# PASSIONLab/ELBA

Hardware: AMD Instinct MI355X
Metric: overlap nnz/sec (A·Aᵀ SpGEMM, SharedSeeds semiring, after Prune(numshared<=1)) (higher is better)
Workload: dtype u32

## Files before the change

elba_amd/csrc/capi.hip:

```cpp
#include "common.hpp"
#include "ov_plan.hpp"
#include <new>

using namespace elba;

struct elba_ctx {
    Ctx c;
};

namespace {

template <class F>
int guarded(elba_ctx *ctx, F &&f)
{
    if (!ctx) return ELBA_ERR_INVALID_ARG;
    try {
        ELBA_HIP(hipSetDevice(ctx->c.device));
        f(ctx->c);
        return ELBA_OK;
    } catch (const Error &e) {
        ctx->c.last_error = e.msg;
        return e.code;
    } catch (const std::bad_alloc &) {
        ctx->c.last_error = "host allocation failed";
// ... 685 lines not shown

int elba_export_kmer_matrix(elba_ctx *ctx, elba_kmer_matrix_t *out)
{
    return guarded(ctx, [&](Ctx &c) {
        ELBA_REQUIRE(out, ELBA_ERR_INVALID_ARG, "export_kmer_matrix: null output");
        memset(out, 0, sizeof(*out));
        ELBA_REQUIRE(has(c.v, P_A), ELBA_ERR_STATE, "export_kmer_matrix: no k-mer matrix");
        const size_t M = (size_t)c.M, N = (size_t)c.N, Z = (size_t)c.Z;
        auto rp = download<uint32_t>(c, c.a_rowptr.p, M + 1);
        auto cp = download<uint32_t>(c, c.a_colptr.p, N + 1);
        auto csr = download<uint64_t>(c, c.a_csr.p, Z);
        auto csc = download<uint64_t>(c, c.a_csc.p, Z);
        out->nrows = c.M; out->ncols = c.N; out->nnz = c.Z;
        out->colptr = host_alloc<int64_t>(N + 1); out->rowptr = host_alloc<int64_t>(M + 1);
        out->csc_row = host_alloc<int64_t>(Z); out->csc_val = host_alloc<uint32_t>(Z);
        out->csr_col = host_alloc<int64_t>(Z); out->csr_val = host_alloc<uint32_t>(Z);
        for (size_t i = 0; i <= N; ++i) out->colptr[i] = cp[i];
        for (size_t i = 0; i <= M; ++i) out->rowptr[i] = rp[i];
        for (size_t z = 0; z < Z; ++z) {
            out->csc_row[z] = (int64_t)(csc[z] >> 32) + c.first_global_id_rows(); out->csc_val[z] = (uint32_t)csc[z];
            out->csr_col[z] = (int64_t)(csr[z] >> 32); out->csr_val[z] = (uint32_t)csr[z] & (c.csr_suffix ? 0xFFFFu : (c.csr_hints ? 0x3FFFFFFFu : 0xFFFFFFFFu));
        }
        if (c.csr_inline) {
            std::vector<size_t> fill(rp.begin(), rp.end() - 1);
            for (size_t k = 0; k < N; ++k)
                for (size_t z = cp[k]; z < cp[k + 1]; ++z) { const size_t at = fill[(size_t)(csc[z] >> 32)]++; out->csr_col[at] = (int64_t)k; out->csr_val[at] = (uint32_t)csc[z]; }
        }
        if (c.A_has_kmers) {
            out->kmers = host_alloc<uint64_t>(N);
            if (N) ELBA_HIP(hipMemcpyAsync(out->kmers, c.rel_kmers.p, N * 8, hipMemcpyDeviceToHost, c.stream));
            if (c.cfg.k > 32) {
                out->kmers_lo = host_alloc<uint64_t>(N);
                if (N) ELBA_HIP(hipMemcpyAsync(out->kmers_lo, c.rel_kmers_lo.p, N * 8, hipMemcpyDeviceToHost, c.stream));
            }
            if (c.cfg.k > 64) {
                out->kmers_lo2 = host_alloc<uint64_t>(N);
                if (N) ELBA_HIP(hipMemcpyAsync(out->kmers_lo2, c.rel_kmers_lo2.p, N * 8, hipMemcpyDeviceToHost, c.stream));
            }
            ELBA_HIP(hipStreamSynchronize(c.stream));
        }
    });
}

void elba_free_kmer_matrix(elba_kmer_matrix_t *m)
{
    if (!m) return;
    free(m->kmers); free(m->kmers_lo); free(m->kmers_lo2); free(m->colptr); free(m->csc_row); free(m->csc_val); free(m->rowptr); free(m->csr_col); free(m->csr_val);
    memset(m, 0, sizeof(*m));
}

int elba_kmer_histogram(elba_ctx *ctx, int64_t *hist, int64_t len)
{
    return guarded(ctx, [&](Ctx &c) {
        ELBA_REQUIRE(hist && len > 0, ELBA_ERR_INVALID_ARG, "kmer_histogram: null output");
        ELBA_REQUIRE(has(c.v, P_A), ELBA_ERR_STATE, "kmer_histogram: no k-mer matrix");
        auto cp = download<uint32_t>(c, c.a_colptr.p, (size_t)c.N + 1);
        for (int64_t i = 0; i < len; ++i) hist[i] = 0;
        for (int64_t k = 0; k < c.N; ++k) { int64_t n = (int64_t)cp[(size_t)k + 1] - cp[(size_t)k]; if (n < len) hist[n]++; }
    });
}

int elba_get_device_view(elba_ctx *ctx, elba_device_view *v)
{
    return guarded(ctx, [&](Ctx &c) {
        ELBA_REQUIRE(v, ELBA_ERR_INVALID_ARG, "get_device_view: null output");
        memset(v, 0, sizeof(*v));
        v->stream = (void *)c.stream;
        if (has(c.v, P_A)) { v->M = c.M; v->N = c.N; v->Z = c.Z; v->a_rowptr = c.a_rowptr.p; v->a_csr = c.a_csr.p; v->a_colptr = c.a_colptr.p; v->a_csc = c.a_csc.p;
                        v->a_csr_format = c.csr_inline ? ELBA_CSR_INLINE : (c.csr_suffix ? ELBA_CSR_DENSE : (c.csr_hints ? ELBA_CSR_HINTS : ELBA_CSR_PLAIN));
                        v->a_csr_pos_mask = c.csr_suffix ? 0xFFFFu : (c.csr_hints ? 0x3FFFFFFFu : 0xFFFFFFFFu);
                        v->a_kmers = c.A_has_kmers ? c.rel_kmers.p : nullptr;
                        v->a_gather_slots = c.use_ell && c.ell_compact ? c.ell_nslots : 0;
                        v->a_slot_kid = c.use_ell && c.ell_compact ? c.ell_slot_kid.p : nullptr; }
        if (has(c.v, P_B)) { v->Y = c.Y; v->b_rowptr = c.b_rowptr.p; v->b_col = c.b_col.p; v->b_val = c.b_val.p; }
    });
}

int elba_set_option(elba_ctx *ctx, const char *name, int64_t value)
{
    return guarded(ctx, [&](Ctx &c) {
        ELBA_REQUIRE(name, ELBA_ERR_INVALID_ARG, "set_option: null name");
        struct { const char *n; bool *b; } flags[] = {
            {"overlap_cold_calls", &c.cold_calls}, {"no_symmetry", &c.opt.no_symmetry}, {"no_ell", &c.opt.no_ell}, {"no_pay", &c.opt.no_pay}, {"mir32", &c.opt.mir32},
            {"no_hints", &c.opt.no_hints}, {"no_sample", &c.opt.no_sample}, {"no_slab", &c.opt.no_slab}, {"no_ell_compact", &c.opt.no_ell_compact}, {"msd_no_rank", &c.opt.msd_no_rank}, {"msd_rank", &c.opt.msd_rank}, {"csr_pairs_late", &c.opt.csr_pairs_late}, {"no_suffix", &c.opt.no_suffix}, {"ov_generic", &c.opt.ov_generic}, {"no_row_order", &c.opt.no_row_order}, {"no_inline", &c.opt.no_inline}, {"panel_inline", &c.opt.panel_inline}, {"kmer_pairs", &c.opt.kmer_pairs},
            {"kmer_unfused", &c.opt.kmer_unfused}, {"kmer_no_msd", &c.opt.kmer_no_msd}, {"kmer_msd", &c.opt.kmer_msd}, {"csr_pairs", &c.opt.csr_pairs}, {"emit_plain", &c.opt.emit_plain}, {"trace", &c.opt.trace}, {"measure_prep", &c.opt.measure_prep}};
        for (auto &f : flags) if (!strcmp(name, f.n)) { *f.b = value != 0; return; }
        if (!strcmp(name, "kmer_drop")) { ELBA_REQUIRE(value >= 0 && value <= 3, ELBA_ERR_INVALID_ARG, "set_option: kmer_drop is 0..3"); c.opt.kmer_drop = (int)value; }
        else if (!strcmp(name, "dense_up")) { ELBA_REQUIRE(value >= 0 && value <= 3, ELBA_ERR_INVALID_ARG, "set_option: dense_up is 0..3"); c.opt.dense_up = (int)value; }
        else if (!strcmp(name, "dense_wgs")) { ELBA_REQUIRE(value >= 1 && value <= 16, ELBA_ERR_INVALID_ARG, "set_option: dense_wgs is 1..16"); c.opt.dense_wgs = (int)value; }
        else if (!strncmp(name, "tune", 4) && name[4] >= '1' && name[4] <= '7' && name[4] != '6' && name[5] == 0) c.opt.tune[name[4] - '0'] = value;
        else if (!strcmp(name, "msd_small_cap")) c.opt.msd_small_cap = (int)value;
        else if (!strcmp(name, "kmer_batch_instances")) { ELBA_REQUIRE(value >= 0, ELBA_ERR_INVALID_ARG, "set_option: kmer_batch_instances is >= 0"); c.opt.kmer_batch_instances = value; }
        else if (!strcmp(name, "msd_wide_bits")) c.opt.msd_wide_bits = (int)value;
        else if (!strcmp(name, "ell_slot_cap")) c.opt.ell_slot_cap = (int)value;
        else if (!strcmp(name, "slab_pct")) { ELBA_REQUIRE(value >= 1 && value <= 1000, ELBA_ERR_INVALID_ARG, "set_option: slab_pct is 1..1000"); c.opt.slab_pct = (int)value; }
        else if (!strcmp(name, "slab_q16")) { ELBA_REQUIRE(value >= 0 && value < (1ll << 31), ELBA_ERR_INVALID_ARG, "set_option: slab_q16 is 0..2^31"); c.opt.slab_q16 = (int)value; }
        else if (!strcmp(name, "dk")) { ELBA_REQUIRE(value == -1 || value == 0 || value == 1 || value == 2 || value == 4, ELBA_ERR_INVALID_ARG, "set_option: dk is -1 (chosen per matrix), 0, 1, 2 or 4"); c.opt.dk = (int)value; }
        else if (!strcmp(name, "aln_tiers")) { ELBA_REQUIRE(value >= 0, ELBA_ERR_INVALID_ARG, "set_option: aln_tiers is a string of the digits 1, 2, 4, 8"); c.opt.aln_tiers = value; }
        else if (!strcmp(name, "aln_wide_hint")) c.opt.aln_wide_hint = (int)value;
        else if (!strcmp(name, "aln_long_hint")) c.opt.aln_long_hint = (int)value;
        else if (!strcmp(name, "polish_trace_bytes")) { ELBA_REQUIRE(value >= 0, ELBA_ERR_INVALID_ARG, "set_option: polish_trace_bytes is >= 0"); c.opt.polish_trace_bytes = value; }
        else throw Error{ELBA_ERR_INVALID_ARG, std::string("set_option: unknown option ") + name};
    });
}

int elba_release_workspace(elba_ctx *ctx)
{
    return guarded(ctx, [&](Ctx &c) {
        ELBA_REQUIRE(!c.dist_owner && c.ov_phase == 0, ELBA_ERR_STATE, "release_workspace: the context holds exchanged records or is inside a sharded multiplication");
        ELBA_HIP(hipStreamSynchronize(c.stream));
        c.ws_a.release(); c.ws_b.release(); c.ws_c.release(); c.ws_d.release(); c.ws_e.release(); c.ws_f.release(); c.ws_g.release(); c.ws_h.release(); c.ws_sort.release();
        c.csr_words.release(); c.kid_of_entry.release();
        c.cg_ptr.release(); c.cg_slot.release(); c.cg_kdeg.release(); c.cg_term.release(); c.cg_vinfo.release(); c.cg_ctr.release();
        c.cg_flag.release(); c.cg_cidx.release(); c.cg_nel.release(); c.cg_eoff.release();
        c.gl_ptr.release(); c.gl_bits.release(); c.gl_cnt.release(); c.gl_off.release(); c.gl_ctr.release(); c.gl_part.release(); c.gl_out.release();
        c.pl_cstart.release(); c.pl_cstrand.release(); c.pl_best.release(); c.pl_rec.release(); c.pl_clen.release(); c.pl_cred.release(); c.pl_ctr.release();
        c.pl_k0.release(); c.pl_k1.release(); c.pl_eptr.release(); c.pl_head.release(); c.pl_hidx.release(); c.pl_delta.release(); c.pl_dsum.release(); c.pl_gstart.release();
        c.pl_tok.release(); c.pl_tpos.release(); c.pl_seg_off.release(); c.pl_seg_start.release(); c.pl_seg_depth.release();
        c.po_plan.release(); c.po_rec.release(); c.po_toff.release(); c.po_trace.release(); c.po_col.release(); c.po_gap.release(); c.po_cnt.release();
        c.po_emit.release(); c.po_off.release(); c.po_cstat.release(); c.po_seq.release(); c.po_seqoff.release(); c.po_ctr.release();
        for (int b = 0; b < 2; ++b) { c.cg_far[b].release(); c.cg_rank[b].release(); c.cg_mn[b].release(); c.cg_cfar[b].release(); c.cg_crank[b].release(); }
        c.pu_k0.release(); c.pu_k1.release(); c.pu_eptr.release(); c.pu_head.release(); c.pu_hidx.release(); c.pu_delta.release();
        c.pu_dsum.release(); c.pu_gstart.release(); c.pu_tok.release(); c.pu_tpos.release(); c.pu_sel.release(); c.pu_rows.release(); c.pu_cols.release(); c.pu_vals.release();
        c.tm_cnt.release(); c.tm_bytes.release(); c.tm_first.release(); c.tm_boff.release(); c.tm_srcb.release();
        c.sg.release();
        c.tp_ntips.release(); c.tp_anchor.release();
        c.bb_end.release(); c.bb_len.release();
        c.wk_best.release(); c.wk_cnt.release(); c.wk_nweak.release(); c.wk_after.release();
        c.br_flank.release();
        c.sr_word.release();
        if (has(c.v, P_COUNTS)) { c.pre_ready = false; c.pre_consumed = true; }
    });
}

int elba_get_stat(elba_ctx *ctx, const char *name, int64_t *value)
{
    return guarded(ctx, [&](Ctx &c) {
        ELBA_REQUIRE(name && value, ELBA_ERR_INVALID_ARG, "get_stat: null name or value");
        if (!strcmp(name, "overlap_mirror_placed")) *value = c.ov_mir_placed;
        else if (!strcmp(name, "overlap_slab_q16")) *value = (int64_t)c.ov_slab_q16_used;
        else if (!strcmp(name, "kmer_path")) *value = c.kmer_path;
        else if (!strcmp(name, "kmer_passes")) *value = c.kmer_passes;
        else if (!strcmp(name, "kmer_crowded_buckets")) *value = c.kmer_crowded;
        else if (!strcmp(name, "kmer_crowded_small")) *value = c.kmer_crowded_small;
        else if (!strcmp(name, "kmer_largest_pass")) *value = c.kmer_largest_pass;
        else if (!strcmp(name, "kmer_peak_bytes")) *value = c.kmer_peak_bytes;
        else if (!strcmp(name, "kmer_buckets")) *value = c.kmer_buckets;
        else if (!strcmp(name, "overlap_passes")) *value = c.ov_passes;
        else if (!strcmp(name, "overlap_spec")) *value = c.ov_spec;
        else if (!strcmp(name, "overlap_forwarded")) *value = c.ov_forwarded;
        else if (!strncmp(name, "overlap_tier_limit_", 19) && name[19] >= '0' && name[19] < '0' + NUM_LDS_TIERS && !name[20]) *value = c.ov_tier_limit[name[19] - '0'];
        else if (!strncmp(name, "overlap_tier_queued_", 20) && name[20] >= '0' && name[20] < '0' + NUM_TIERS && !name[21]) *value = c.ov_tier_queued[name[20] - '0'];
        else if (!strncmp(name, "overlap_tier_done_", 18) && name[18] >= '0' && name[18] < '0' + NUM_TIERS && !name[19]) *value = c.ov_tier_done[name[18] - '0'];
        else if (!strcmp(name, "overlap_sort_rows_bucket")) *value = c.ov_sort_rows[0];
        else if (!strcmp(name, "overlap_sort_rows_huge")) *value = c.ov_sort_rows[1];
        else if (!strcmp(name, "overlap_family")) *value = c.ov_family;
        else if (!strcmp(name, "overlap_pay16")) *value = c.ov_pay16;
        else if (!strcmp(name, "overlap_rec16")) *value = c.ov_rec16_used;
        else if (!strcmp(name, "matrix_col_stride")) *value = has(c.v, P_A) && c.use_ell ? (int64_t)c.s_stride : 0;
        else if (!strcmp(name, "matrix_fbits")) *value = has(c.v, P_A) ? (int64_t)c.fbits : 0;
        else if (!strcmp(name, "matrix_pos16")) *value = has(c.v, P_A) && c.pos16 ? 1 : 0;
        else if (!strcmp(name, "matrix_hints")) *value = has(c.v, P_A) && c.csr_hints ? 1 : 0;
        else if (!strcmp(name, "matrix_inline")) *value = has(c.v, P_A) && c.csr_inline ? 1 : 0;
        else if (!strcmp(name, "matrix_suffix")) *value = has(c.v, P_A) && c.csr_suffix ? 1 : 0;
        else if (!strcmp(name, "matrix_csr_words")) *value = has(c.v, P_A) && c.csr_one_word ? 1 : 0;
        else if (!strcmp(name, "spgemm_prep_us")) *value = c.prep_us;
        else if (!strcmp(name, "emit_us")) *value = c.emit_us;
        else if (!strcmp(name, "triples_path")) *value = c.triples_path;
        else if (!strcmp(name, "text_tile_bytes")) *value = TEXT_TILE_BYTES;
        else if (!strcmp(name, "text_scan_span")) *value = scan_block_span();
        else if (!strcmp(name, "padded_columns")) *value = has(c.v, P_A) && c.use_ell ? 1 : 0;
        else if (!strcmp(name, "gather_slots")) *value = has(c.v, P_A) && c.use_ell ? c.ell_nslots : 0;
        else if (!strcmp(name, "contig_count")) *value = has(c.v, P_S, P_CONTIGS) ? c.cstats.contigs : 0;
        else if (!strcmp(name, "contig_cycles")) *value = has(c.v, P_S, P_CONTIGS) ? c.cstats.cycles : 0;
        else if (!strcmp(name, "contig_circular")) *value = has(c.v, P_S, P_CONTIGS) ? c.cg_circular : 0;
        else if (!strcmp(name, "contig_singletons")) *value = has(c.v, P_S, P_CONTIGS) ? c.cg_singletons : 0;
        else if (!strcmp(name, "contig_reads")) *value = has(c.v, P_S, P_CONTIGS) ? c.cstats.contig_reads : 0;
        else if (!strcmp(name, "contig_bases")) *value = has(c.v, P_S, P_CONTIGS) ? c.cstats.bases : 0;
        else if (!strcmp(name, "contig_branches")) *value = has(c.v, P_S, P_CONTIGS) ? c.cstats.branches : 0;
        else if (!strncmp(name, "graph_", 6)) {
            const bool ok = has(c.v, P_S, P_CONTIGS) && c.gl_for == c.cg_serial;
            const elba_graph_stats &g = c.gstats;
            const char *f = name + 6;
            int64_t x;
            if (!strcmp(f, "segments")) x = g.segments; else if (!strcmp(f, "candidates")) x = g.candidates; else if (!strcmp(f, "links")) x = g.links;
            else if (!strcmp(f, "closures")) x = g.closures; else if (!strcmp(f, "twisted")) x = g.twisted; else if (!strcmp(f, "unplaced")) x = g.unplaced;
            else if (!strcmp(f, "clamped")) x = g.clamped; else if (!strcmp(f, "asymmetric")) x = g.asymmetric;
            else throw Error{ELBA_ERR_INVALID_ARG, std::string("get_stat: unknown counter ") + name};
            *value = ok ? x : 0;
        }
        else if (!strncmp(name, "place_", 6)) {
            const bool ok = has(c.v, P_S, P_CONTIGS) && c.pl_for == c.cg_serial && c.pl_for != 0;
            const elba_place_stats &g = c.plstats;
            const char *f = name + 6;
            int64_t x;
            if (!strcmp(f, "chain")) x = g.chain; else if (!strcmp(f, "anchored")) x = g.anchored; else if (!strcmp(f, "unanchored")) x = g.unanchored;
            else if (!strcmp(f, "skipped")) x = g.skipped; else if (!strcmp(f, "candidates")) x = g.candidates; else if (!strcmp(f, "clipped")) x = g.clipped;
            else if (!strcmp(f, "outside")) x = g.outside; else if (!strcmp(f, "wrapped")) x = g.wrapped; else if (!strcmp(f, "segments")) x = g.segments;
            else if (!strcmp(f, "max_depth")) x = g.max_depth;
            else throw Error{ELBA_ERR_INVALID_ARG, std::string("get_stat: unknown counter ") + name};
            *value = ok ? x : 0;
        }
        else if (!strncmp(name, "polish_", 7)) {
            const bool ok = has(c.v, P_S, P_CONTIGS) && c.po_for == c.cg_serial && c.po_for != 0;
            const elba_polish_stats &g = c.postats;
            const char *f = name + 7;
            int64_t x;
            if (!strcmp(f, "voted")) x = g.voted; else if (!strcmp(f, "rejected")) x = g.rejected; else if (!strcmp(f, "outside")) x = g.outside;
            else if (!strcmp(f, "low_depth_columns")) x = g.low_depth_columns; else if (!strcmp(f, "bases_before")) x = g.bases_before;
            else if (!strcmp(f, "bases_after")) x = g.bases_after; else if (!strcmp(f, "sum_dist")) x = g.sum_dist; else if (!strcmp(f, "cells")) x = g.cells;
            else if (!strcmp(f, "batches")) x = g.batches;
            else throw Error{ELBA_ERR_INVALID_ARG, std::string("get_stat: unknown counter ") + name};
            *value = ok ? x : 0;
        }
        else if (!strcmp(name, "contig_rank_us")) *value = has(c.v, P_S, P_CONTIGS) ? (int64_t)(c.cstats.ms_rank * 1000.0f) : -1;
        else if (!strcmp(name, "resident_bytes_A")) {
            int64_t b = 0;
            if (has(c.v, P_A)) {
                b = (int64_t)(c.M + 1) * 4 + (int64_t)(c.N + 1) * 4 + 16 * c.Z;
                if (c.use_ell) b += 8 * c.ell_nslots * (int64_t)c.s_stride + (c.ell_compact ? 4 * c.ell_nslots : 0);
                if (c.csr_suffix) b += (4ll * c.N) << c.j_shift;
            }
            *value = b;
        }
        else throw Error{ELBA_ERR_INVALID_ARG, std::string("get_stat: unknown counter ") + name};
    });
}

int elba_kmer_hash_owner(elba_ctx *ctx, const uint64_t *kmers, int64_t n, int nprocs, uint64_t *hash, int32_t *owner)
{
    return guarded(ctx, [&](Ctx &c) { stage_ref_hash_owner(c, kmers, n, nprocs, hash, owner); });
}
// ... 133 lines not shown
```

elba_amd/csrc/common.hpp:

```cpp
#pragma once
#include <hip/hip_runtime.h>
#include <cstdint>
#include <cstdio>
#include <cstdlib>
#include <cstring>
#include <mutex>
#include <string>
#include <vector>
#include "../../include/elba_amd.h"
#include "state.hpp"
#include "msd_plan.hpp"

namespace elba {

struct Error {
    int code;
    std::string msg;
};

#define ELBA_HIP(expr)                                                                                   \
    do {                                                                                                 \
        hipError_t e__ = (expr);                                                                         \
        if (e__ != hipSuccess) {                                                                         \
            throw ::elba::Error{e__ == hipErrorOutOfMemory ? ELBA_ERR_OUT_OF_MEMORY : ELBA_ERR_HIP,      \
// ... 41 lines not shown
        if (e != hipSuccess) { want = bytes; e = hipMalloc(&p, want); }
        if (e != hipSuccess) { p = nullptr; throw Error{ELBA_ERR_OUT_OF_MEMORY, "hipMalloc of " + std::to_string(bytes) + " bytes failed"}; }
        cap = want;
    }
    void reserve_exact(size_t bytes)
    {
        if (bytes <= cap) return;
        release();
        const hipError_t e = hipMalloc(&p, bytes);
        if (e != hipSuccess) { p = nullptr; throw Error{ELBA_ERR_OUT_OF_MEMORY, "hipMalloc of " + std::to_string(bytes) + " bytes failed"}; }
        cap = bytes;
    }
    template <class T> T *as() const { return reinterpret_cast<T *>(p); }
    void swap(DevBuf &o) { void *tp = p; p = o.p; o.p = tp; size_t tc = cap; cap = o.cap; o.cap = tc; }
};

struct EventTimer {
    hipEvent_t a = nullptr, b = nullptr;
    void init() { if (!a) { ELBA_HIP(hipEventCreate(&a)); ELBA_HIP(hipEventCreate(&b)); } }
    void start(hipStream_t s) { init(); ELBA_HIP(hipEventRecord(a, s)); }
    void stop(hipStream_t s) { ELBA_HIP(hipEventRecord(b, s)); }
    float ms() { float t = 0; ELBA_HIP(hipEventSynchronize(b)); ELBA_HIP(hipEventElapsedTime(&t, a, b)); return t; }
    ~EventTimer() { if (a) (void)hipEventDestroy(a); if (b) (void)hipEventDestroy(b); }
};

template <int N>
struct PhaseMarks {
    hipEvent_t e[N] = {};
    void mark(int k, hipStream_t s) { if (!e[k]) ELBA_HIP(hipEventCreate(&e[k])); ELBA_HIP(hipEventRecord(e[k], s)); }
    float ms(int from, int to) { float t = 0; ELBA_HIP(hipEventSynchronize(e[to])); ELBA_HIP(hipEventElapsedTime(&t, e[from], e[to])); return t; }
    ~PhaseMarks() { for (int k = 0; k < N; ++k) if (e[k]) (void)hipEventDestroy(e[k]); }
};

void exclusive_scan_u32(hipStream_t s, const uint32_t *in, uint32_t *out, int64_t n, DevBuf &tmp);
void exclusive_scan_u32_to_i64(hipStream_t s, const uint32_t *in, int64_t *out, int64_t n, DevBuf &tmp);
__device__ __forceinline__ uint32_t column_hint(const uint64_t *col, uint32_t L, uint32_t i, uint32_t win_lo, uint32_t win_hi)
{
    bool own_g = false, own_w = false;
    uint32_t mult = 0;
    for (uint32_t t = 0; t < L; ++t) {
        const uint32_t j = (uint32_t)(col[t] >> 32);
        if (j == i) { ++mult; continue; }
        const bool par = ((i ^ j) & 1u) ? j < i : j > i;
        own_g |= par; own_w |= par || j < win_lo || j >= win_hi;
    }
    if (mult >= 2) return 0u;
    return (own_g ? 0u : 1u) | (own_w ? 0u : 2u);
}

int radix_sort_pairs(hipStream_t s, uint64_t *k0, uint64_t *v0, uint64_t *k1, uint64_t *v1, int64_t n, int bit_lo, int bit_hi, DevBuf &tmp);
int radix_sort_keys(hipStream_t s, uint64_t *k0, uint64_t *k1, int64_t n, int bit_lo, int bit_hi, DevBuf &tmp, bool first_hist_done = false);
int radix_sort_where(int64_t n, int bit_lo, int bit_hi);
struct CsrFin { int idbits, pb, rs, mb, pbi; uint64_t *csr; uint32_t *rowptr; int64_t M; };
void radix_sort_keys_to_csr(hipStream_t s, uint64_t *k0, uint64_t *k1, int64_t n, const CsrFin &f, DevBuf &tmp);
int radix_sort_pairs_k32(hipStream_t s, uint32_t *k0, uint64_t *v0, uint32_t *k1, uint64_t *v1, int64_t n, int bit_lo, int bit_hi, DevBuf &tmp);
void group_offsets_k32(hipStream_t s, const uint32_t *sorted_keys, int64_t n, uint32_t *ptr, int64_t nkeys);
void radix_column_scan(hipStream_t s, uint32_t *rows, int64_t nrows, uint32_t nbins, DevBuf &tmp);
uint32_t *radix_first_histogram(int64_t n, int bit_lo, int bit_hi, DevBuf &tmp, int *shift, int *bits, int *tile);
void fill_u32(hipStream_t s, uint32_t *p, uint32_t v, int64_t n);
void fill_u64(hipStream_t s, uint64_t *p, uint64_t v, int64_t n);
void group_offsets_u32(hipStream_t s, const uint64_t *sorted_keys, int key_shift, int64_t n, uint32_t *ptr, int64_t nkeys);
uint64_t reduce_max_u64(hipStream_t s, const uint64_t *p, int64_t n, DevBuf &tmp);
int64_t scan_block_span();

struct Options {
    bool no_symmetry = false;
    bool no_ell = false;
    bool no_pay = false;
    bool mir32 = false;
    bool no_hints = false;
    bool no_sample = false;
    bool no_ell_compact = false;
    bool no_slab = false;
    bool csr_pairs_late = false;
    bool msd_rank = false;
    bool msd_no_rank = false;
    int ell_slot_cap = 0;
    int slab_pct = 175;
    int slab_q16 = 0;
    bool panel_inline = false;
    bool no_inline = false;
    bool no_suffix = false;
    bool ov_generic = false;
    bool no_row_order = false;
    bool kmer_pairs = false;
    bool kmer_unfused = false;
    bool kmer_msd = false;
    bool kmer_no_msd = false;
    bool csr_pairs = false;
    bool emit_plain = false;
    bool trace = false;
    bool measure_prep = false;
    int64_t tune[8] = {0, 0, 0, 0, 0, 0, 0, 0};
    int msd_wide_bits = 0;
    int64_t kmer_batch_instances = 0;
    int msd_small_cap = 0;
    int kmer_drop = 0;
    int dense_up = 1;
    int dense_wgs = 8;
    int dk = -1;
    int64_t aln_tiers = 0;
    int aln_wide_hint = 6, aln_long_hint = 6000;
    int64_t polish_trace_bytes = 0;
};

struct RowWindow { int64_t lo, hi; int64_t rows() const { return hi - lo; } };

struct alignas(16) SymEntry { uint32_t col; int32_t suffix, suffixT; uint32_t meta; };
static_assert(sizeof(SymEntry) == 16, "tr.hip and stars.hip read 16-byte entries");

struct Ctx {
    elba_cfg cfg{};
    Options opt;
    int device = 0;
    hipStream_t stream = nullptr;
    std::string last_error;
    int num_cus = 256;
    Validity v;

    int64_t nreads = 0, first_global_id = 0, packed_bytes = 0;
    const uint8_t *d_packed = nullptr;
    const uint64_t *d_byte_off = nullptr;
    const uint32_t *d_len = nullptr;
    DevBuf own_packed, own_byte_off, own_len;
    uint32_t max_read_len = 0;
    std::vector<uint32_t> h_len;
    std::vector<uint64_t> h_byte_off;
    bool tx_index = false;
    DevBuf tx_recs, tx_name_pos, tx_name_len;
    std::vector<elba_fasta_record_t> tx_h_recs; std::vector<uint64_t> tx_h_name_pos; std::vector<uint32_t> tx_h_name_len;

    int triples_path = 0;
    int kmer_passes = 1;
    int64_t kmer_crowded = 0, kmer_crowded_small = 0, kmer_largest_pass = 0;
    int64_t kmer_peak_bytes = 0;
    int64_t kmer_buckets = 0;
    int kmer_path = 0;
    int64_t I = 0, ndistinct = 0;
    DevBuf inst_off;
    DevBuf rel_kmers;
    DevBuf rel_kmers_lo;
    DevBuf rel_kmers_lo2;
    DevBuf rel_counts;
    DevBuf csr_words;
    bool pre_pairs = false;
    bool pre_ready = false, pre_consumed = false, pre_words = false, pre_hints = false, pre_hints_done = false, pre_ell_done = false, pre_inline = false, pre_inline_pending = false ; int pre_rs = 0, pre_pbi = 0; int pre_nb = 0, pre_pb = 0; uint64_t pre_maxpos = 0;
    bool csr_hints = false, ov_hints_used = false, ov_rec16 = false;
    bool csr_inline = false;
    bool csr_inline_window = false;
    bool csr_one_word = false;
    bool csr_suffix = false;
    DevBuf ov_sample;
    int64_t A_products = 0;
    DevBuf prod_ctr;
    DevBuf kid_of_entry;
    elba_kmer_stats kstats{};

    bool A_has_kmers = false;
    int64_t M = 0, N = 0, Z = 0, max_row_nnz = 0, max_col_nnz = 0;
    DevBuf a_rowptr, a_csr, a_colptr, a_csc;
    DevBuf a_ell;
    bool use_ell = false;
    bool ell_compact = false;
    int64_t ell_nslots = 0, ell_cap_cols = 0;
    DevBuf ell_slot_kid;
    DevBuf a_ellj;
// ... 32 lines not shown
    DevBuf tr_in_rows, tr_in_cols, tr_in_vals;
    int64_t tr_M = 0, tr_nnz = 0, tr_id_base = 0;
    DevBuf tr_deg, tr_pas, tr_flags, tr_k0, tr_v0, tr_k1, tr_v1, tr_ptr, tr_sym, tr_src, tr_mark, tr_ctr, tr_sel, tr_out_rows, tr_out_cols, tr_out_vals;
    int64_t tr_sym_M = 0, tr_sym_n = 0;
    elba_string_stats sstats{};

    int64_t cg_n = 0, cg_E = 0, cg_bases = 0, cg_circular = 0, cg_singletons = 0;
    DevBuf cg_ptr, cg_slot, cg_kdeg, cg_far[2], cg_rank[2], cg_mn[2], cg_term, cg_vinfo, cg_flag, cg_cidx, cg_nel, cg_eoff, cg_ctr;
    DevBuf cg_cid, cg_eread, cg_epre, cg_estr, cg_eboff, cg_soff, cg_coff, cg_seq, cg_kind;
    DevBuf cg_cfar[2], cg_crank[2];
    EventTimer cg_t_total, cg_t_rank;
    elba_contig_stats cstats{};

    DevBuf gl_ptr, gl_bits, gl_cnt, gl_off, gl_ctr, gl_part, gl_out;
    EventTimer gl_t_total;
    elba_graph_stats gstats{};
    uint64_t cg_serial = 0, gl_for = 0;

    int64_t pu_M = 0, pu_n = 0, pu_nseg = 0;
    DevBuf pu_k0, pu_k1, pu_eptr, pu_head, pu_hidx, pu_delta, pu_dsum, pu_gstart, pu_tok, pu_tpos, pu_ctr, pu_sel, pu_rows, pu_cols, pu_vals;
    DevBuf pu_seg_off, pu_seg_start, pu_seg_depth, pu_trim, pu_flags;
    EventTimer pu_t_total;
    elba_pileup_stats pustats{};
    elba_pileup_cfg pu_cfg{};

    DevBuf pl_cstart, pl_cstrand, pl_best, pl_rec, pl_clen, pl_cred, pl_ctr;
    DevBuf pl_k0, pl_k1, pl_eptr, pl_head, pl_hidx, pl_delta, pl_dsum, pl_gstart, pl_tok, pl_tpos, pl_seg_off, pl_seg_start, pl_seg_depth;
    EventTimer pl_t_total;
    elba_place_stats plstats{};
    uint64_t pl_for = 0;

    DevBuf po_plan, po_rec, po_toff, po_trace, po_col, po_gap, po_cnt, po_emit, po_off, po_cstat, po_seq, po_seqoff, po_ctr;
    EventTimer po_t_total, po_t_align;
    elba_polish_stats postats{};
    uint64_t po_for = 0;

    int64_t tm_n = 0, tm_packed_bytes = 0;
    DevBuf tm_packed, tm_off, tm_len, tm_src, tm_beg, tm_end;
    DevBuf tm_cnt, tm_bytes, tm_first, tm_boff, tm_srcb, tm_ctr;
    EventTimer tm_t_total, tm_t_repack;
    elba_trim_stats tmstats{};

    struct SgWork {
        DevBuf ptr, removed, keep, pos, st, rows, cols, vals;
        EventTimer t_total, t_compact;
        void release() { ptr.release(); removed.release(); keep.release(); pos.release(); st.release(); rows.release(); cols.release(); vals.release(); }
    } sg;

    DevBuf tp_ntips, tp_anchor;
    elba_tip_stats tpstats{};

    DevBuf bb_end, bb_len;
    elba_bubble_stats bbstats{};

    DevBuf wk_best, wk_cnt, wk_nweak, wk_after;
    elba_weak_stats wkstats{};

    DevBuf br_flank;
    elba_bridge_stats brstats{};

    DevBuf sr_word;
    elba_star_stats srstats{};

    DevBuf ws_scan, ws_sort, ws_a, ws_b, ws_c, ws_d, ws_e, ws_f;
    DevBuf ws_cursor;
    DevBuf ws_g, ws_h;
    DevBuf ov_totcnt, ov_mir, ov_tmp, ov_sum_tmp;
    bool ov_low_clean = false;
    DevBuf ov_rowcnt, ov_rowoff, ov_lists, ov_counters, ov_gtable, ov_sortkeys;
    int64_t ov_tmp_cap = 0;
    bool ov_sort_used[2] = {false, false};
    bool ov_tiers_known = false, ov_tier_used[8] = {false, false, false, false, false, false, false, false};
    int64_t b_cap_entries = 0;
    uint64_t ov_calls = 0;
    uint32_t ov_prior_q16 = 0;
    uint32_t ov_slab_q16 = 0;
    DevBuf ov_slab;
    int64_t ov_slab_cap = 0;
    DevBuf ov_tickrows;
    DevBuf ov_slabpos, ov_slabn;
    bool ov_slab_on = false;
    uint32_t ov_slab_q16_used = 0;
    int64_t ov_mir_placed = 0;
    int64_t ov_spec = 0;
    int64_t ov_tier_limit[5] = {0, 0, 0, 0, 0}, ov_tier_queued[6] = {0, 0, 0, 0, 0, 0}, ov_tier_done[6] = {0, 0, 0, 0, 0, 0}, ov_sort_rows[2] = {0, 0};
    int64_t ov_family = 0, ov_pay16 = 0, ov_rec16_used = 0;
    int64_t ov_passes = 0, ov_forwarded = 0;
    int ov_phase = 0;
    int ov_pend_passes = 1; bool ov_pend_timed = false; float ov_pend_ms[3] = {0, 0, 0};
    std::vector<uint64_t> ov_remote_bounds;
    DevBuf ov_remote;
    int64_t ov_send_slot = 0;
    DevBuf ov_cursors;
    bool own_stream = true;

    EventTimer t_total, t_a, t_b, t_c;
    EventTimer t_emit, t_emit_plain; int64_t prep_us = -1, emit_us = -1;
    struct PinnedHost { void *p = nullptr; size_t cap = 0; void reserve(size_t n) { if (n <= cap) return; if (p) (void)hipHostFree(p); p = nullptr; cap = 0; ELBA_HIP(hipHostMalloc(&p, n, hipHostMallocDefault)); cap = n; } ~PinnedHost() { if (p) (void)hipHostFree(p); } };
    PinnedHost ov_host;
    PhaseMarks<5> ov_marks;
};

inline void reads_replaced(Ctx &c, Event ev)
{
    done(c.v, ev);
    if (c.A_has_kmers) done(c.v, EV_MATRIX_OF_OLD_READS);
    c.tx_index = false;
}

struct GraphInput { int64_t M, n, id_base; const int64_t *rows, *cols; const elba_overlap_t *vals; };
inline GraphInput graph_input(Ctx &c, const char *who)
{
    if (has(c.v, P_EDGES)) return {c.tr_in_M, c.tr_in_n, 0, c.tr_in_rows.as<int64_t>(), c.tr_in_cols.as<int64_t>(), c.tr_in_vals.as<elba_overlap_t>()};
    ELBA_REQUIRE(has(c.v, P_ALN), ELBA_ERR_STATE, std::string(who) + ": no overlaps (call elba_align_seeds or elba_set_overlaps)");
    ELBA_REQUIRE(c.row_hi < 0 || (c.row_lo == 0 && c.row_hi == c.M), ELBA_ERR_STATE,
                 std::string(who) + ": this context aligned a row shard; gather the ranks' overlaps and load them with elba_set_overlaps");
    return {c.M, c.naln, c.first_global_id_rows(), c.aln_rows.as<int64_t>(), c.aln_cols.as<int64_t>(), c.aln_out.as<elba_overlap_t>()};
}

struct ReadSource { const uint8_t *packed; const uint64_t *byte_off; const uint32_t *len; bool replicated; };
inline ReadSource read_source(Ctx &c, int64_t M, const char *who, const char *what, bool take_replicated = true)
{
    if (take_replicated && c.aln_all_n == M && c.aln_all_n >= 0) return {c.aln_all_packed.as<uint8_t>(), c.aln_all_off.as<uint64_t>(), c.aln_all_len.as<uint32_t>(), true};
    if (has(c.v, P_READS) && c.nreads == M) return {c.d_packed, c.d_byte_off, c.d_len, false};
    std::string w(what);
    w.replace(w.find('#'), 1, std::to_string(M));
    throw Error{ELBA_ERR_STATE, std::string(who) + ": the " + w + " are not on this context (elba_set_reads or elba_dist_set_all_reads)"};
}

struct DepthBufs { DevBuf &k0, &k1, &eptr, &head, &hidx, &delta, &dsum, &gstart, &tok, &tpos, &seg_off, &seg_start, &seg_depth; };
void depth_reserve(const DepthBufs &b, int64_t max_keys, int64_t G);
const uint64_t *depth_segments(Ctx &c, const DepthBufs &b, int64_t E, int64_t M, int mb, int pb, const uint32_t *len, unsigned long long *ctr);

constexpr int PLACE_CTR_BAD = 2, PLACE_CTR_WORDS = 16;
struct PlaceWork { GraphInput in; ReadSource src; int64_t M, base, E, nc; elba_placement_t *rec; unsigned long long *ctr; const uint32_t *clen; };
PlaceWork place_records(Ctx &c, int skip_flags, const char *who, bool depth_bufs, EventTimer *t);
[[noreturn]] void place_throw_bad_pair(Ctx &c, const PlaceWork &w, int64_t a, const char *who);

void stage_set_reads_fasta(Ctx &c, const char *chunk, int64_t chunk_bytes, uint64_t chunk_file_offset, const elba_fasta_record_t *recs, int64_t nreads,
                           int64_t first_global_id, elba_ingest_stats *stats);
void launch_fasta_encode(Ctx &c, const uint8_t *d_chunk, uint64_t chunk_file_offset, uint64_t chunk_bytes, const elba_fasta_record_t *d_recs, const uint64_t *d_byte_off,
                         int64_t nreads, uint8_t *d_packed);
constexpr uint32_t TEXT_TILE_BYTES = 4096;
void stage_set_reads_text(Ctx &c, const char *chunk, int64_t chunk_bytes, uint64_t chunk_file_offset, const elba_text_cfg *cfg, elba_text_stats *stats);
void stage_export_read_index(Ctx &c, elba_fasta_record_t *recs, uint64_t *name_pos, uint32_t *name_len, int64_t nreads_capacity);
void stage_count_kmers(Ctx &c);
void stage_create_kmer_matrix(Ctx &c);
bool msd_matrix_from_triples(Ctx &c, int64_t M, int64_t N, int64_t Z, const int64_t *d_rows, const int64_t *d_cols, const uint32_t *d_vals);
bool msd_count_kmers(Ctx &c, uint64_t I, elba_kmer_stats &st);
void choose_column_store(Ctx &c, int64_t N, int64_t max_col);
void stage_set_kmer_matrix(Ctx &c, int64_t M, int64_t N, int64_t Z, const int64_t *rows, const int64_t *cols, const uint32_t *vals);
void stage_set_kmer_matrix_device(Ctx &c, int64_t M, int64_t N, int64_t Z, const int64_t *d_rows, const int64_t *d_cols, const uint32_t *d_vals);
void stage_export_triples_device(Ctx &c, int64_t *d_rows, int64_t *d_cols, uint32_t *d_vals);
void stage_create_seed_matrix(Ctx &c);
void stage_seed_matrix_begin(Ctx &c, int nranks, const uint64_t *bounds_host, uint64_t *send_counts_host);
void stage_seed_matrix_fill(Ctx &c, void *d_send, const uint64_t *offsets_host);
void stage_seed_matrix_end(Ctx &c, const void *d_recv, int64_t nrecv);
void stage_seed_matrix_send(Ctx &c, int nranks, const uint64_t *bounds_host, void *d_send, int64_t slot);
bool stage_seed_matrix_recv(Ctx &c, void *d_recv, int64_t slot, int64_t *slot_needed);
void stage_align_seeds(Ctx &c, int mat, int mis, int gap, int dropoff);
void stage_dist_set_all_reads(Ctx &c, const void *d_packed, int64_t packed_bytes, const void *d_byte_off, const void *d_len, int64_t nreads_total);
void stage_set_overlaps(Ctx &c, int64_t nreads, const int64_t *rows, const int64_t *cols, const elba_overlap_t *vals, int64_t n);
void stage_transitive_reduction(Ctx &c, double bad_read_cutoff, int fuzz);
void stage_generate_contigs(Ctx &c, int flags);
void stage_generate_contigs_ex(Ctx &c, const elba_contig_cfg *cfg);
void stage_export_assembly_links(Ctx &c, elba_links_t *out);
// ... 28 lines not shown
```

elba_amd/csrc/ov_plan.hpp:

```cpp
#pragma once
#include <algorithm>
#include <cstddef>
#include <cstdint>

namespace elba {

constexpr int NUM_LDS_TIERS = 5;
constexpr int NUM_TIERS = NUM_LDS_TIERS + 1;
constexpr int LDS_TBITS0 = 9;
constexpr uint32_t STAGE_CHUNK = 1024;
constexpr uint32_t STAGE_REC_BYTES = 32;
constexpr uint32_t FIN_WAVE2_MAX = 1024;
constexpr uint32_t SLAB_PAD = 16;
constexpr int RP_TILE = 1024;
constexpr int FIN_HUGE_BLOCKS = 32;
constexpr int OV_SAMPLE_ROWS = 256, OV_SAMPLE_TIER = 3;
constexpr size_t OV_LDS_MAX = 160 * 1024;

namespace ov_spec {
constexpr uint32_t half = 1, inl = 1, pay16 = 1, rec16 = 1, suffix = 0, qblk_log2 = 0, j_shift = 0;
constexpr uint32_t hint_mask = 1u << 31, pos_mask = 0x3FFFFFFFu;
}

enum OvFamily { OV_DENSE, OV_PAY, OV_S32, OV_SHARED };
constexpr int OV_GRID_DENSE_WGS = 0, OV_GRID_SPILL = -1;
struct OvTierRow { OvFamily family; int tier, block, tbits, tbc, cu_factor, slot_bytes; bool global, payload, dense; int dense_up_min; };
constexpr OvTierRow OV_ROWS[] = {
    {OV_DENSE, 0, 256, 9, 9, OV_GRID_DENSE_WGS, 18, false, false, true, 0},
    {OV_DENSE, 1, 256, 10, 0, 4, 18, false, false, true, 0},
    {OV_DENSE, 1, 512, 10, 10, 4, 18, false, false, true, 1},
    {OV_DENSE, 2, 512, 11, 0, 2, 18, false, false, true, 0},
    {OV_DENSE, 2, 1024, 11, 11, 2, 18, false, false, true, 2},
    {OV_DENSE, 3, 1024, 12, 0, 1, 18, false, false, true, 0},
    {OV_PAY, 0, 128, 9, 0, 9, 26, false, true, false, 0},
    {OV_PAY, 1, 256, 10, 0, 4, 26, false, true, false, 0},
    {OV_PAY, 2, 512, 11, 0, 2, 26, false, true, false, 0},
    {OV_PAY, 3, 1024, 12, 0, 1, 26, false, true, false, 0},
    {OV_S32, 0, 128, 9, 0, 12, 18, false, false, false, 0},
    {OV_S32, 1, 256, 10, 0, 7, 18, false, false, false, 0},
    {OV_S32, 2, 512, 11, 0, 3, 18, false, false, false, 0},
    {OV_S32, 3, 1024, 12, 0, 1, 18, false, false, false, 0},
    {OV_SHARED, 4, 256, 13, 0, 1, 18, false, false, false, 0},
    {OV_SHARED, NUM_LDS_TIERS, 256, 0, 0, OV_GRID_SPILL, 0, true, false, false, 0},
};
constexpr int OV_NROWS = (int)(sizeof(OV_ROWS) / sizeof(OV_ROWS[0]));

constexpr int64_t ov_stage_slack(int num_cus) { return (int64_t)num_cus * 32 * STAGE_CHUNK + 64; }

constexpr size_t ov_row_lds(const OvTierRow &r, bool pay16)
{
    const size_t waves = (size_t)(r.block / 64), table = r.global ? 0 : (size_t)r.slot_bytes << r.tbits;
    return table + 256 + waves * (r.dense ? 2368 : r.global ? 2560 : r.payload ? 3072 : pay16 ? 2048 : 2560);
}

inline int ov_row_of(OvFamily family, int tier, int dense_up)
{
    int found = -1;
    for (int r = 0; r < OV_NROWS; ++r) {
        const OvTierRow &x = OV_ROWS[r];
        if (x.tier == tier && (x.family == family || x.family == OV_SHARED) && dense_up >= x.dense_up_min) found = r;
    }
    return found;
}

struct OvOptions {
    bool no_symmetry = false, no_pay = false, mir32 = false, no_slab = false, no_sample = false, ov_generic = false;
    int dk = -1, dense_up = 1, dense_wgs = 8, slab_q16 = 0, slab_pct = 175;
    int64_t tune3 = 0, tune4 = 0, tune5 = 0, tune7 = 0;
};
struct OvHints { uint32_t prior_q16 = 0, slab_q16 = 0; bool tiers_known = false, tier_used[NUM_TIERS] = {false, false, false, false, false, false}, sort_used[2] = {false, false}; };
struct OvInput {
    int64_t M = 0, N = 0, Z = 0, row_lo = 0, row_hi = 0, max_row_nnz = 0, max_col_nnz = 0;
    uint32_t fbits = 1;
    bool pos16 = false, use_ell = false, csr_hints = false, csr_inline = false, csr_suffix = false, have_row_order = false;
    int num_cus = 256;
    OvOptions opt;
    OvHints hints;
    int phase = 0, pass = 1;
    int64_t tmp_cap = 0, free_bytes = 0, workspace_hint_bytes = 0;
};

struct OvLaunch { int row = -1, grid = 0, block = 0; size_t lds = 0; };
struct OvFinPlan {
    int64_t nrows = 0;
    bool slabs = false, scan_rowptr = false, narrow = false;
    int slab_fold_blocks = 0, rowptr_blocks = 0, row_blocks = 0, bucket_blocks = 0, huge_blocks = FIN_HUGE_BLOCKS;
    uint64_t sort_stride = 2;
    uint32_t sorts = 0;
};
struct OvPlan {
    int64_t nrows = 0;
    bool whole = false, ell = false, forced = false;
    uint32_t half = 0, pos_mask = 0, hint_mask = 0, suffix = 0, inl = 0;
    bool row_order = false, hints_used = false;
    bool pay = false, pay16 = false;
    OvFamily family = OV_S32;
    int dk = 1;
    bool spec = false;
    uint32_t min_tier = 0, qblk_log2 = 0, prior_q16 = 16384, use_feedback = 1, max_col = 1;
    unsigned long long fb_enough = 0;
    uint32_t nsample = 0, sstep = 1;
    bool slab_on = false; int64_t slab_cap = 0; uint32_t slab_prior_q16 = 0;
    uint64_t gstride = 2; int spill_blocks = 64;
    int64_t slack = 0, tmp_cap = 0, b_cap = 0;
    bool mir16 = false;
    uint32_t tier_limit[NUM_LDS_TIERS] = {0, 0, 0, 0, 0};
    OvLaunch tier[NUM_TIERS], sample;
    int tmax = NUM_TIERS;
    uint32_t launched = 0;
    int zero_blocks_max = 0, classify_blocks = 0;
    OvFinPlan fin;
};

inline bool ov_spec_ok(const OvPlan &p)
{
    return !p.forced && p.dk == 0 && !p.pay && (p.pay16 ? 1u : 0u) == ov_spec::pay16 && p.ell && p.half == ov_spec::half && p.hint_mask == ov_spec::hint_mask &&
           p.pos_mask == ov_spec::pos_mask && p.inl == ov_spec::inl && (p.mir16 ? 1u : 0u) == ov_spec::rec16 && p.suffix == ov_spec::suffix && !p.row_order &&
           p.qblk_log2 == ov_spec::qblk_log2 && p.whole;
}

inline OvLaunch ov_launch_of(int row, bool pay16, int num_cus, int dense_wgs, int spill_blocks)
{
    const OvTierRow &r = OV_ROWS[row];
    OvLaunch l;
    l.row = row; l.block = r.block; l.lds = ov_row_lds(r, pay16);
    l.grid = r.cu_factor == OV_GRID_SPILL ? spill_blocks : num_cus * (r.cu_factor == OV_GRID_DENSE_WGS ? dense_wgs : r.cu_factor);
    return l;
}

inline OvFinPlan plan_ov_finalize(const OvInput &in, bool slabs, bool all_sorts, bool remote)
{
    OvFinPlan f;
    const int64_t M = in.M, cus = in.num_cus;
    f.nrows = in.row_hi - in.row_lo;
    f.slabs = slabs;
    f.slab_fold_blocks = slabs && f.nrows > 0 ? (int)((f.nrows + 255) / 256) : 0;
    while (f.sort_stride < (uint64_t)M) f.sort_stride <<= 1;
    f.scan_rowptr = M + 1 > (1 << 17);
    f.rowptr_blocks = (int)(f.scan_rowptr ? (M + 1 + 255) / 256 : (M + 1 + RP_TILE - 1) / RP_TILE);
    if (f.nrows <= 0) return f;
    f.row_blocks = (int)std::min<int64_t>((f.nrows + 3) / 4, cus * 32);
    f.narrow = in.opt.tune4 != 2 && !remote &&
               std::min<uint64_t>((uint64_t)std::max<int64_t>(in.max_row_nnz, 1) * (uint64_t)std::max<int64_t>(in.max_col_nnz, 1), (uint64_t)M) <= (uint64_t)FIN_WAVE2_MAX;
    f.bucket_blocks = (int)std::min<int64_t>(f.nrows, cus * 4);
    if (!f.narrow && (all_sorts || in.hints.sort_used[0])) f.sorts |= 1u;
    if (!f.narrow && (all_sorts || in.hints.sort_used[1])) f.sorts |= 2u;
    return f;
}

inline bool ov_one_triangle(const OvInput &in) { return in.phase >= 1 || !in.opt.no_symmetry || in.csr_inline; }

struct OvSpill { uint64_t gstride; int blocks; };
inline OvSpill ov_spill_tables(int64_t M, int num_cus)
{
    OvSpill s{2, 0};
    while (s.gstride < 2ull * (uint64_t)(M > 1 ? M : 1)) s.gstride <<= 1;
    s.blocks = (int)((4ull << 30) / (20ull * s.gstride));
    s.blocks = s.blocks < 64 ? 64 : (s.blocks > num_cus * 2 ? num_cus * 2 : s.blocks);
    return s;
}

inline void ov_plan_capacities(const OvInput &in, OvPlan &p)
{
    const int64_t M = in.M, Z = in.Z;
    const bool half = ov_one_triangle(in);
    const OvSpill sp = ov_spill_tables(M, in.num_cus);
    p.gstride = sp.gstride; p.spill_blocks = sp.blocks;
    p.slack = ov_stage_slack(in.num_cus);
    p.tmp_cap = in.tmp_cap;
    if (p.tmp_cap == 0) {
        if (in.workspace_hint_bytes > 0) p.tmp_cap = in.workspace_hint_bytes / (int64_t)STAGE_REC_BYTES;
        else {
            const int64_t budget = (int64_t)((size_t)in.free_bytes / 2 / (STAGE_REC_BYTES + (half ? 2 * (24 + 32) : 24)));
            p.tmp_cap = std::min<int64_t>(std::max<int64_t>(half ? Z / 2 : Z, 1 << 16) + p.slack, std::max<int64_t>(budget, 1024));
        }
        if (p.tmp_cap < 1024) p.tmp_cap = 1024;
    }
    p.b_cap = half ? 2 * p.tmp_cap : p.tmp_cap;
}

inline void ov_plan_switches(const OvInput &in, OvPlan &p)
{
    const OvOptions &o = in.opt;
    const int64_t Z = in.Z, nrows = p.nrows;
    p.max_col = (uint32_t)(in.max_col_nnz > 0 ? in.max_col_nnz : 1);
    p.half = in.phase >= 1 ? 2u : (ov_one_triangle(in) ? 1u : 0u);
    p.pos_mask = in.csr_suffix ? 0xFFFFu : (in.csr_hints ? 0x3FFFFFFFu : 0xFFFFFFFFu);
    p.hint_mask = !in.csr_hints ? 0u : (p.half == 2u ? 1u << 30 : (p.half == 1u ? 1u << 31 : 0u));
    p.suffix = in.csr_suffix && p.half == 1u ? 1u : 0u;
    p.inl = in.csr_inline ? 1u : 0u;
    p.row_order = p.suffix && in.have_row_order;
    p.hints_used = p.hint_mask != 0u || p.suffix != 0u || in.csr_inline;
    p.prior_q16 = in.hints.prior_q16 ? in.hints.prior_q16 : 16384u;
    p.use_feedback = in.hints.prior_q16 ? 0u : 1u;
    p.fb_enough = (unsigned long long)std::min<int64_t>(std::max<int64_t>(Z / 32, 1 << 16), 1 << 23);
    p.pay = in.pos16 && !o.no_pay;
    p.pay16 = p.pay && in.use_ell && !in.csr_suffix && o.tune3 != 1 && ((uint64_t)in.max_row_nnz << in.fbits) <= 65536ull;
    if (p.pay16) p.pay = false;
    p.family = p.suffix ? OV_DENSE : p.pay ? OV_PAY : OV_S32;
    p.mir16 = in.pos16 && !o.mir32;
    p.qblk_log2 = o.tune5 > 0 ? (uint32_t)std::min<int64_t>(o.tune5 - 1, 12) : 0u;
    p.min_tier = (p.pay16 && nrows >= 65536 && Z / nrows >= 1024 && o.tune4 != 1) ? 2u : 0u;
    if (o.tune7 >= 1 && o.tune7 <= NUM_TIERS) p.min_tier = (uint32_t)(o.tune7 - 1);
    p.dk = o.dk >= 0 ? o.dk : ((in.csr_inline && in.N > 0 && Z < 3 * in.N) ? 0 : 1);
    p.spec = ov_spec_ok(p);
}

inline void ov_plan_sample_slabs(const OvInput &in, OvPlan &p)
{
    const OvOptions &o = in.opt;
    const int64_t M = in.M, nrows = p.nrows;
    const bool sampling = p.use_feedback && nrows >= 8192 && !o.no_sample;
    p.nsample = sampling ? (uint32_t)OV_SAMPLE_ROWS : 0u; p.sstep = sampling ? (uint32_t)(nrows / OV_SAMPLE_ROWS) : 1u;
    p.slab_prior_q16 = o.slab_q16 > 0 ? (uint32_t)o.slab_q16 : in.hints.slab_q16;
    p.slab_on = in.phase == 0 && p.half == 1u && p.mir16 && !o.no_slab && nrows > 0 && (sampling || p.slab_prior_q16 != 0u);
    if (p.slab_on) {
        p.slab_cap = std::min<int64_t>(p.tmp_cap + (int64_t)SLAB_PAD * nrows, 0xFFFF0000ll);
        if (p.slab_cap + M >= 0xFFFFFFFFll) p.slab_cap = std::max<int64_t>(0xFFFFFFFFll - M - 1, 0);
        if (p.slab_cap <= (int64_t)SLAB_PAD * nrows + 1) p.slab_on = false;
    }
}

inline void ov_plan_tiers(const OvInput &in, OvPlan &p)
{
    const OvOptions &o = in.opt;
    const int64_t M = in.M, nrows = p.nrows;
    for (int t = 0; t < NUM_TIERS; ++t) p.tier[t] = ov_launch_of(ov_row_of(p.family, t, (int)o.dense_up), p.pay16, in.num_cus, o.dense_wgs, p.spill_blocks);
    for (int t = 0; t < NUM_LDS_TIERS; ++t) {
        const uint32_t T = 1u << OV_ROWS[p.tier[t].row].tbits;
        p.tier_limit[t] = std::min((T >> 2) * 3, T - (uint32_t)p.tier[t].block) - 1;
    }
    if (p.nsample) p.sample = p.tier[OV_SAMPLE_TIER];
    if (o.tune4 != 2 && in.pass == 1) {
        const uint64_t ubm = std::min<uint64_t>((uint64_t)std::max<int64_t>(in.max_row_nnz, 1) * (uint64_t)p.max_col, (uint64_t)(uint32_t)M);
        const int gmax = ubm <= 1 ? 1 : 64 - __builtin_clzll(2 * ubm - 1);
        p.tmax = gmax <= LDS_TBITS0 ? 0 : gmax - LDS_TBITS0;
        p.tmax = std::max(p.tmax, (int)p.min_tier);
        if (p.suffix) p.tmax = std::max(p.tmax, (int)o.dense_up);
    }
    const bool all_tiers = !in.hints.tiers_known || in.phase == 2;
    for (int t = 0; t < NUM_TIERS; ++t)
        if (nrows > 0 && (all_tiers || in.hints.tier_used[t]) && t <= p.tmax) p.launched |= 1u << t;
}

inline OvPlan plan_ov(const OvInput &in)
{
    OvPlan p;
    const OvOptions &o = in.opt;
    const int64_t cus = in.num_cus, nrows = in.row_hi - in.row_lo;
    p.nrows = nrows;
    p.whole = in.row_lo == 0 && in.row_hi == in.M;
    p.ell = in.use_ell;
    p.forced = o.ov_generic || o.dk >= 0 || o.tune3 != 0 || o.tune4 != 0 || o.tune5 != 0 || o.tune7 != 0;
    ov_plan_capacities(in, p);
    ov_plan_switches(in, p);
    ov_plan_sample_slabs(in, p);
    ov_plan_tiers(in, p);
    p.zero_blocks_max = in.num_cus * 8;
    p.classify_blocks = nrows > 0 ? (int)std::min<int64_t>((nrows + 255) / 256, cus * 4) : 0;
    p.fin = plan_ov_finalize(in, p.half == 1u && p.mir16 && p.slab_on, !in.hints.tiers_known, false);
    return p;
}

inline OvInput ov_next_pass(const OvInput &in, const OvPlan &p, bool overflow, unsigned long long cursor)
{
    OvInput n = in;
    n.pass = in.pass + 1;
    n.tmp_cap = overflow ? (int64_t)cursor + p.slack : p.tmp_cap;
    n.hints.tiers_known = false;
    return n;
}

struct OvMeasured { int64_t Z = 0, nnz = 0, ndiag = 0, extra_nnz = 0; bool whole = false; unsigned long long fb_claims = 0, fb_ub = 0; unsigned int tier_count[NUM_TIERS] = {0, 0, 0, 0, 0, 0}, fin_count[2] = {0, 0}; };
inline OvHints ov_next_hints(const OvHints &old, const OvMeasured &m)
{
    OvHints h = old;
    for (int t = 0; t < NUM_TIERS; ++t) h.tier_used[t] = m.tier_count[t] > 0;
    h.tiers_known = true;
    h.sort_used[0] = m.fin_count[0] > 0; h.sort_used[1] = m.fin_count[1] > 0;
    if (m.whole && m.Z > 0 && m.extra_nnz == 0) {
        const double r = 0.5 * (double)(m.nnz - m.ndiag) / (double)m.Z * 65536.0;
        h.slab_q16 = r < 1.0 ? 1u : (r > 4.0e9 ? 4000000000u : (uint32_t)r);
    }
    if (m.fb_ub > 0) {
        const double r = 1.25 * (double)m.fb_claims / (double)m.fb_ub * 65536.0;
        const uint32_t q = r < 64.0 ? 64u : (r > 4.0e9 ? 4000000000u : (uint32_t)r);
        if (old.prior_q16 == 0 || q > old.prior_q16 + old.prior_q16 / 10 || q + old.prior_q16 / 10 < old.prior_q16) h.prior_q16 = q;
    }
    return h;
}

}
```

elba_amd/csrc/spgemm.hip:

```cpp
#include "common.hpp"
#include "ov_plan.hpp"
#include <algorithm>
#include <string>
#include <type_traits>
#include <utility>

namespace elba {

namespace {

constexpr uint32_t EMPTY = 0xFFFFFFFFu;
constexpr uint32_t FIN_WAVE_MAX = 256;
constexpr uint32_t FIN_LDS_MAX = 4096;

struct alignas(128) OvShard {
    unsigned long long yraw, nnz, ndiag, nupper, fb_claims, fb_ub, products;
    unsigned int maxshared;
    unsigned int tier_done[NUM_TIERS];
};
constexpr int NUM_SHARDS = 64;

struct OvCounters {
    unsigned long long cursor;
    unsigned long long products;
// ... 39 lines not shown
    uint32_t M;
    uint32_t Mcols;
    uint32_t row_lo, row_hi;
    uint32_t fbits;
    uint32_t half;
    uint32_t tier_limit[NUM_LDS_TIERS];
    uint32_t use_feedback;
    uint32_t prior_q16;
    uint32_t *row_cnt;
    uint32_t *low_cnt;
    unsigned long long *row_off;
    uint32_t *lists;
    const uint32_t *row_order, *row_label;
    uint32_t *sample_list; uint32_t nsample, sstep;
    uint32_t *fin_lists;
    OvCounters *ctr;
    StageRec *tmp; unsigned long long tmp_cap;
    uint32_t rec16; uint4 *rec; uint32_t *tick;
    uint32_t *gtable; unsigned long long gstride;
    uint4 *slab; unsigned long long slab_cap; uint32_t slab_prior_q16, slab_pct;
    unsigned long long *slab_pos;
};

struct OvSpecParams {
    static constexpr uint32_t half = ov_spec::half, inl = ov_spec::inl, pay16 = ov_spec::pay16, rec16 = ov_spec::rec16, suffix = ov_spec::suffix, qblk_log2 = ov_spec::qblk_log2, j_shift = ov_spec::j_shift;
    static constexpr uint32_t hint_mask = ov_spec::hint_mask, pos_mask = ov_spec::pos_mask;
    static constexpr uint32_t row_lo = 0, row_hi = 0xFFFFFFFFu;
    static constexpr const uint32_t *a_colptr = nullptr, *a_ellj = nullptr, *row_order = nullptr, *row_label = nullptr;
    static constexpr const uint64_t *a_csc = nullptr;
    static constexpr StageRec *tmp = nullptr;
    static constexpr uint32_t *gtable = nullptr;
    static constexpr unsigned long long gstride = 0;
    const uint32_t *a_rowptr; const uint64_t *a_csr; const uint64_t *a_ell;
    uint32_t *tick_rows;
    uint32_t s_stride, lpc_log2, max_col, fbits, M, Mcols, use_feedback;
    uint32_t tier_limit[NUM_LDS_TIERS];
    unsigned long long fb_enough, tmp_cap;
    uint32_t *row_cnt, *low_cnt; unsigned long long *row_off;
    uint32_t *lists, *sample_list;
    OvCounters *ctr;
    uint4 *rec; uint32_t *tick;
    uint4 *slab; unsigned long long *slab_pos;
};

struct ZeroList { uint32_t *p[6]; size_t words[6]; int n; };
__global__ __launch_bounds__(256) void k_zero_regions(ZeroList z)
{
    const size_t stride = (size_t)gridDim.x * 256u;
    for (int q = 0; q < z.n; ++q)
        for (size_t i = (size_t)blockIdx.x * 256u + threadIdx.x; i < z.words[q]; i += stride) z.p[q][i] = 0u;
}

struct __attribute__((packed, aligned(4))) RowPair { uint32_t a, b; };
__device__ __forceinline__ uint32_t slab_base(uint32_t rp, uint32_t rp0, uint32_t row_rel, uint32_t q16)
{
    return (uint32_t)(((unsigned long long)(rp - rp0) * q16) >> 16) + SLAB_PAD * row_rel;
}

__device__ __forceinline__ uint32_t wave_sum_u32(uint32_t v)
{
#pragma unroll
    for (int d = 32; d >= 1; d >>= 1) v += __shfl_xor(v, d, 64);
    return v;
}

__device__ __forceinline__ uint32_t guaranteed_tbits(uint32_t ub, uint32_t mcols)
{
    const uint32_t need = ub < mcols ? ub : mcols;
    return need <= 1 ? 1u : (uint32_t)(32 - __clz(2 * need - 1));
}

#include "spgemm_table.hpp"
#include "spgemm_direct.hpp"

struct FinParams {
    const uint32_t *row_cnt; uint32_t *low_cnt; const unsigned long long *row_off; int64_t *b_rowptr;
    const StageRec *tmp; StageRec *mir;
    uint32_t rec16; const uint4 *rec; const uint32_t *tick;
    uint32_t *b_col; elba_seed_t *b_val;
    uint32_t M, row_lo, row_hi, half;
    uint32_t *fin_lists; OvCounters *ctr;
    uint64_t *sortkeys; unsigned long long sort_stride;
    uint32_t *sum_tmp;
    long long b_cap;
    uint32_t mir16;
    const uint32_t *tick_rows;
    const uint32_t *a_rowptr; uint4 *slab;
    const unsigned long long *slab_pos; uint32_t *slab_n;
};

struct SlabCall { uint32_t q16, rp0; };
__device__ __forceinline__ SlabCall slab_call(const FinParams &p)
{
    SlabCall s{0u, 0u};
    if (p.slab) { s.q16 = p.ctr->slab_q16; if (s.q16) s.rp0 = p.a_rowptr[p.row_lo]; }
    return s;
}
__device__ __forceinline__ uint2 slab_row(const FinParams &p, const SlabCall &s, uint32_t i)
{
    if (!s.q16) return make_uint2(0u, 0u);
    return make_uint2(slab_base(p.a_rowptr[i], s.rp0, i - p.row_lo, s.q16), p.slab_n[i]);
}
__global__ void k_slab_fold(FinParams p)
{
    const uint32_t i = p.row_lo + blockIdx.x * blockDim.x + threadIdx.x;
    if (i >= p.row_hi) return;
    const SlabCall s = slab_call(p);
    uint32_t n = 0;
    if (s.q16) {
        const unsigned long long w = p.slab_pos[i];
        const uint32_t base = slab_base(p.a_rowptr[i], s.rp0, i - p.row_lo, s.q16), cur = (uint32_t)w, lim = (uint32_t)(w >> 32);
        n = (cur < lim ? cur : lim) - base;
    }
    p.slab_n[i] = n;
}

__device__ __forceinline__ void fin_load(const FinParams &p, uint32_t low, unsigned long long off, int64_t dst, uint32_t t, uint4 &a, uint4 &b, uint2 sl = make_uint2(0u, 0u))
{
    if (t >= low) {
        if (p.rec16) {
            const uint4 m = p.rec[off + (t - low)];
            a = make_uint4(m.x, 0xFFFFFFFFu, m.y & 0xFFFFu, m.y >> 16); b = make_uint4(m.z & 0xFFFFu, m.z >> 16, m.w, 0u);
        } else { const StageRec *r = &p.tmp[off + (t - low)]; a = r->a; b = r->b; }
    }
    else if (p.mir16) {
        const uint4 m = t < sl.y ? p.slab[sl.x + t] : reinterpret_cast<const uint4 *>(p.mir)[dst + t - sl.y];
        a = make_uint4(m.x, 0xFFFFFFFFu, m.y & 0xFFFFu, m.y >> 16); b = make_uint4(m.z & 0xFFFFu, m.z >> 16, m.w, 0u);
    } else { const StageRec *r = &p.mir[dst + t]; a = r->a; b = r->b; }
}
__device__ __forceinline__ uint32_t fin_col(const FinParams &p, uint32_t low, unsigned long long off, int64_t dst, uint32_t t, uint2 sl = make_uint2(0u, 0u))
{
    if (t >= low) return p.rec16 ? p.rec[off + (t - low)].x : p.tmp[off + (t - low)].a.x;
    return p.mir16 ? (t < sl.y ? p.slab[sl.x + t].x : reinterpret_cast<const uint4 *>(p.mir)[dst + t - sl.y].x) : p.mir[dst + t].a.x;
}
__device__ __forceinline__ elba_seed_t rec_seed(const uint4 a, const uint4 b)
{
    elba_seed_t v;
    v.q0 = a.z; v.t0 = a.w; v.q1 = b.x; v.t1 = b.y; v.numshared = (int32_t)b.z;
    return v;
}

__global__ __launch_bounds__(256) void k_row_pointers(FinParams p)
{
    __shared__ unsigned long long wsum[4], bsum;
    const uint32_t tid = threadIdx.x, lane = tid & 63, w = tid >> 6;
    const uint32_t n = p.M + 1, t0 = blockIdx.x * RP_TILE;
    unsigned long long pre = 0;
    {
        const uint4 *ca = reinterpret_cast<const uint4 *>(p.row_cnt), *cb = reinterpret_cast<const uint4 *>(p.low_cnt), *cc = reinterpret_cast<const uint4 *>(p.slab_n);
#pragma unroll 4
        for (uint32_t q = tid; q < t0 / 4; q += 256) {
            const uint4 x = ca[q], z = cb[q];
            pre += (unsigned long long)x.x + x.y + x.z + x.w + z.x + z.y + z.z + z.w;
            if (cc) { const uint4 y2 = cc[q]; pre += (unsigned long long)y2.x + y2.y + y2.z + y2.w; }
        }
    }
    uint32_t v[4];
    unsigned long long mine = 0;
#pragma unroll
    for (int u = 0; u < 4; ++u) {
        const uint32_t e = t0 + tid * 4 + u;
        v[u] = e < p.M ? p.row_cnt[e] + p.low_cnt[e] + (p.slab_n ? p.slab_n[e] : 0u) : 0u;
        mine += v[u];
    }
#pragma unroll
    for (int d = 32; d >= 1; d >>= 1) pre += __shfl_xor(pre, d, 64);
    unsigned long long inc = mine;
#pragma unroll
    for (int d = 1; d < 64; d <<= 1) { const unsigned long long o = __shfl_up(inc, d, 64); if ((int)lane >= d) inc += o; }
    if (lane == 63) wsum[w] = inc;
    if (tid == 0) bsum = 0;
    __syncthreads();
    if (lane == 0) atomicAdd(&bsum, pre);
    __syncthreads();
    unsigned long long run = bsum + inc - mine;
    for (uint32_t k = 0; k < w; ++k) run += wsum[k];
#pragma unroll
    for (int u = 0; u < 4; ++u) {
        const uint32_t e = t0 + tid * 4 + u;
        if (e < n) p.b_rowptr[e] = (int64_t)run;
        run += v[u];
    }
}

__global__ void k_sum_counts(FinParams p)
{
    const uint32_t e = blockIdx.x * blockDim.x + threadIdx.x;
    if (e <= p.M) p.sum_tmp[e] = e < p.M ? p.row_cnt[e] + p.low_cnt[e] + (p.slab_n ? p.slab_n[e] : 0u) : 0u;
}

__global__ __launch_bounds__(256) void k_mirror(FinParams p)
{
    const uint32_t lane = threadIdx.x & 63;
    const uint32_t wave = (blockIdx.x * blockDim.x + threadIdx.x) >> 6;
    const uint32_t nwaves = (gridDim.x * blockDim.x) >> 6;
    uint32_t placed = 0;
    for (uint32_t i = p.row_lo + wave; i < p.row_hi; i += nwaves) {
        const uint32_t own = p.row_cnt[i];
        const unsigned long long off = p.row_off[i];
        const uint32_t y = own + p.low_cnt[i] + (p.slab_n ? p.slab_n[i] : 0u);
        if (lane == 0 && y > FIN_WAVE2_MAX) {
            const int which = y > FIN_LDS_MAX ? 1 : 0;
            const uint32_t at = atomicAdd(&p.ctr->fin_count[which], 1u);
            p.fin_lists[(size_t)which * p.M + at] = i;
        }
        if (!p.half || p.rec16) continue;
        if (p.tick_rows && !((p.tick_rows[i >> 5] >> (i & 31u)) & 1u)) continue;
        for (uint32_t t = lane; t < own; t += 64) {
            const uint4 a = p.tmp[off + t].a;
            if (a.y == 0xFFFFFFFFu) continue;
            const uint4 b = p.tmp[off + t].b;
            const int64_t at = p.b_rowptr[a.x] + (int64_t)a.y;
            if (at >= p.b_cap) continue;
            if (p.mir16) reinterpret_cast<uint4 *>(p.mir)[at] = make_uint4(i, a.w | a.z << 16, b.y | b.x << 16, b.z);
            else {
                p.mir[at].a = make_uint4(i, 0xFFFFFFFFu, a.w, a.z);
                p.mir[at].b = make_uint4(b.y, b.x, b.z, 0u);
            }
        }
    }
    if (p.half && p.rec16) {
        const uint32_t n = p.ctr->ntick, stride = gridDim.x * blockDim.x;
        for (uint32_t e = blockIdx.x * blockDim.x + threadIdx.x; e < n; e += stride) {
            const uint32_t i = p.tick[3ull * e], t = p.tick[3ull * e + 1u], tk = p.tick[3ull * e + 2u];
            const uint4 r = p.rec[p.row_off[i] + t];
            const uint4 img = make_uint4(i, (r.y >> 16) | (r.y << 16), (r.z >> 16) | (r.z << 16), r.w);
            ++placed;
            const int64_t at = p.b_rowptr[r.x] + (int64_t)tk;
            if (at >= p.b_cap) continue;
            if (p.mir16) reinterpret_cast<uint4 *>(p.mir)[at] = img;
            else { p.mir[at].a = make_uint4(i, 0xFFFFFFFFu, img.y & 0xFFFFu, img.y >> 16); p.mir[at].b = make_uint4(img.z & 0xFFFFu, img.z >> 16, img.w, 0u); }
        }
    }
    placed = wave_sum_u32(placed);
    if (lane == 0 && placed) atomicAdd(&p.ctr->mir_placed, (unsigned long long)placed);
}

__global__ __launch_bounds__(256) void k_finalize_wave(FinParams p)
{
    __shared__ uint32_t colsm[4][FIN_WAVE_MAX];
    const int lane = threadIdx.x & 63, w = threadIdx.x >> 6;
    const uint32_t wave = (blockIdx.x * blockDim.x + threadIdx.x) >> 6;
    const uint32_t nwaves = (gridDim.x * blockDim.x) >> 6;
    uint32_t *cols = colsm[w];
    const SlabCall sc = slab_call(p);
    for (uint32_t i = p.row_lo + wave; i < p.row_hi; i += nwaves) {
        const int64_t dst = p.b_rowptr[i];
        const uint32_t y = (uint32_t)(p.b_rowptr[i + 1] - dst);
        const uint32_t lowt = p.low_cnt[i];
        if (lane == 0 && lowt) p.low_cnt[i] = 0;
        if (y == 0 || y > FIN_WAVE_MAX) continue;
        if (dst + (int64_t)y > p.b_cap) continue;
        const unsigned long long off = p.row_off[i];
        const uint2 sl = slab_row(p, sc, i);
        const uint32_t low = lowt + sl.y;
        uint32_t mine[4];
        uint4 ra[4], rb[4];
#pragma unroll
        for (int u = 0; u < 4; ++u) {
            const uint32_t t = (uint32_t)lane + 64u * u;
            mine[u] = 0xFFFFFFFFu;
            if (t < y) {
                fin_load(p, low, off, dst, t, ra[u], rb[u], sl);
                mine[u] = ra[u].x;
                cols[t] = mine[u];
            }
        }
        __builtin_amdgcn_fence(__ATOMIC_RELEASE, "wavefront");
        __builtin_amdgcn_wave_barrier();
        uint32_t rank[4] = {0, 0, 0, 0};
        for (uint32_t l = 0; l < y; ++l) {
            const uint32_t c = cols[l];
#pragma unroll
            for (int u = 0; u < 4; ++u) rank[u] += c < mine[u] ? 1u : 0u;
        }
#pragma unroll
        for (int u = 0; u < 4; ++u) {
            const uint32_t t = (uint32_t)lane + 64u * u;
            if (t < y) { p.b_col[dst + rank[u]] = mine[u]; p.b_val[dst + rank[u]] = rec_seed(ra[u], rb[u]); }
        }
        __builtin_amdgcn_wave_barrier();
    }
}

__global__ __launch_bounds__(256) void k_finalize_mid(FinParams p)
{
    __shared__ uint64_t lkeys[4][FIN_WAVE2_MAX];
    __shared__ uint32_t bst[4][128], bfl[4][128];
    const int lane = threadIdx.x & 63, w = threadIdx.x >> 6;
// ... 280 lines not shown
{
    uint32_t lo = 0, hi = p.nranks;
    while (hi - lo > 1) { const uint32_t mid = (lo + hi) >> 1; if (p.bounds[mid] <= read) lo = mid; else hi = mid; }
    return lo;
}
template <bool FILL>
__global__ __launch_bounds__(256) void k_remote_mirror(RemoteParams p, unsigned long long *cnt_or_cursor, StageRec *send)
{
    __shared__ uint32_t cnt[REMOTE_MAX_RANKS], fill[REMOTE_MAX_RANKS];
    __shared__ unsigned long long base[REMOTE_MAX_RANKS];
    const uint32_t tid = threadIdx.x, lane = tid & 63, w = tid >> 6;
    const uint32_t r0 = p.row_lo + blockIdx.x * REMOTE_ROWS_PER_BLOCK, r1 = min(r0 + (uint32_t)REMOTE_ROWS_PER_BLOCK, p.row_hi);
    if (tid < REMOTE_MAX_RANKS) { cnt[tid] = 0; fill[tid] = 0; }
    __syncthreads();
    for (uint32_t i = r0 + w; i < r1; i += 4) {
        const uint32_t n = p.row_cnt[i];
        const unsigned long long off = p.row_off[i];
        for (uint32_t t = lane; t < n; t += 64) {
            const uint32_t j = p.rec16 ? p.rec[off + t].x : p.tmp[off + t].a.x;
            if (j != i && (j < p.row_lo || j >= p.row_hi)) atomicAdd(&cnt[remote_rank_of(p, j)], 1u);
        }
    }
    __syncthreads();
    if (tid < p.nranks && cnt[tid]) {
        const unsigned long long b = atomicAdd(&cnt_or_cursor[tid], (unsigned long long)cnt[tid]);
        if (FILL) base[tid] = b;
    }
    if (!FILL) return;
    __syncthreads();
    for (uint32_t i = r0 + w; i < r1; i += 4) {
        const uint32_t n = p.row_cnt[i];
        const unsigned long long off = p.row_off[i];
        for (uint32_t t = lane; t < n; t += 64) {
            uint4 a, b = make_uint4(0u, 0u, 0u, 0u);
            if (p.rec16) { const uint4 m = p.rec[off + t]; a = make_uint4(m.x, 0u, m.y & 0xFFFFu, m.y >> 16); b = make_uint4(m.z & 0xFFFFu, m.z >> 16, m.w, 0u); }
            else a = p.tmp[off + t].a;
            const uint32_t j = a.x;
            if (j != i && (j < p.row_lo || j >= p.row_hi)) {
                if (!p.rec16) b = p.tmp[off + t].b;
                const uint32_t d = remote_rank_of(p, j);
                const unsigned long long at = base[d] + atomicAdd(&fill[d], 1u);
                send[at].a = make_uint4(j, i, a.w, a.z);
                send[at].b = make_uint4(b.y, b.x, b.z, 0u);
            }
        }
    }
}

__global__ void k_ingest_remote(StageRec *rem, unsigned long long n, uint32_t *low_cnt, uint32_t row_lo, uint32_t row_hi, unsigned long long *bad, unsigned long long *nupper)
{
    const unsigned long long r = (unsigned long long)blockIdx.x * blockDim.x + threadIdx.x;
    unsigned long long up = 0;
    if (r < n) {
        const uint32_t j = rem[r].a.x;
        if (j < row_lo || j >= row_hi) atomicAdd(bad, 1ull);
        else { rem[r].b.w = atomicAdd(&low_cnt[j], 1u); up = rem[r].a.y > j ? 1u : 0u; }
    }
#pragma unroll
    for (int d = 32; d >= 1; d >>= 1) up += __shfl_xor(up, d, 64);
    if ((threadIdx.x & 63) == 0 && up) atomicAdd(nupper, up);
}

__global__ void k_place_remote(FinParams p, const StageRec *rem, unsigned long long n, unsigned long long slot)
{
    if (slot) { rem += (unsigned long long)blockIdx.y * slot; n = (unsigned long long)rem->a.x + 1; if (n > slot) n = slot; }
    for (unsigned long long r = (unsigned long long)blockIdx.x * blockDim.x + threadIdx.x + (slot ? 1 : 0); r < n; r += (unsigned long long)gridDim.x * blockDim.x) {
        const uint4 a = rem[r].a, b = rem[r].b;
        if (a.x < p.row_lo || a.x >= p.row_hi) continue;
        const int64_t at = p.b_rowptr[a.x] + (int64_t)b.w;
        if (at >= p.b_cap) continue;
        if (p.mir16) reinterpret_cast<uint4 *>(p.mir)[at] = make_uint4(a.y, a.z | a.w << 16, b.x | b.y << 16, b.z);
        else { p.mir[at].a = make_uint4(a.y, 0xFFFFFFFFu, a.z, a.w); p.mir[at].b = make_uint4(b.x, b.y, b.z, 0u); }
    }
}


static bool ov_mir16(const Ctx &c) { return c.pos16 && !c.opt.mir32; }

static OvInput ov_input(Ctx &c, int phase, int pass)
{
    OvInput in;
    const RowWindow w = c.window();
    in.M = c.M; in.N = c.N; in.Z = c.Z; in.row_lo = w.lo; in.row_hi = w.hi; in.max_row_nnz = c.max_row_nnz; in.max_col_nnz = c.max_col_nnz;
    in.fbits = c.fbits; in.pos16 = c.pos16; in.use_ell = c.use_ell; in.csr_hints = c.csr_hints; in.csr_inline = c.csr_inline; in.csr_suffix = c.csr_suffix;
    in.have_row_order = c.have_row_order; in.num_cus = c.num_cus;
    const Options &o = c.opt;
    in.opt.no_symmetry = o.no_symmetry; in.opt.no_pay = o.no_pay; in.opt.mir32 = o.mir32; in.opt.no_slab = o.no_slab; in.opt.no_sample = o.no_sample; in.opt.ov_generic = o.ov_generic;
    in.opt.dk = o.dk; in.opt.dense_up = o.dense_up; in.opt.dense_wgs = o.dense_wgs; in.opt.slab_q16 = o.slab_q16; in.opt.slab_pct = o.slab_pct;
    in.opt.tune3 = o.tune[3]; in.opt.tune4 = o.tune[4]; in.opt.tune5 = o.tune[5]; in.opt.tune7 = o.tune[7];
    in.hints.prior_q16 = c.ov_prior_q16; in.hints.slab_q16 = c.ov_slab_q16; in.hints.tiers_known = c.ov_tiers_known;
    for (int t = 0; t < NUM_TIERS; ++t) in.hints.tier_used[t] = c.ov_tier_used[t];
    in.hints.sort_used[0] = c.ov_sort_used[0]; in.hints.sort_used[1] = c.ov_sort_used[1];
    in.phase = phase; in.pass = pass;
    in.tmp_cap = c.ov_tmp_cap; in.workspace_hint_bytes = c.cfg.workspace_hint_bytes;
    if (in.tmp_cap == 0 && in.workspace_hint_bytes <= 0) {
        size_t free_b = 0, total_b = 0;
        ELBA_HIP(hipMemGetInfo(&free_b, &total_b));
        in.free_bytes = (int64_t)free_b;
    }
    return in;
}

template <int R, int DK, bool SPEC> static constexpr auto ov_row_kernel()
{
    constexpr OvTierRow r = OV_ROWS[R];
    if constexpr (r.dense) return &k_spgemm_direct<r.block, false, false, 2, true, r.tbc>;
    else if constexpr (SPEC) return &k_spgemm_direct<r.block, false, false, 0, false, 0, true>;
    else return &k_spgemm_direct<r.block, r.global, r.payload, DK>;
}
template <int R> static constexpr bool ov_row_has_spec() { return !OV_ROWS[R].dense && !OV_ROWS[R].global && !OV_ROWS[R].payload; }
template <int R, typename F> static void ov_row_kernels(F &&f)
{
    f(ov_row_kernel<R, 0, false>());
    if constexpr (!OV_ROWS[R].dense) { f(ov_row_kernel<R, 1, false>()); f(ov_row_kernel<R, 2, false>()); f(ov_row_kernel<R, 4, false>()); }
    if constexpr (ov_row_has_spec<R>()) f(ov_row_kernel<R, 0, true>());
}
template <int... R> static void ov_set_attributes(std::integer_sequence<int, R...>)
{
    (ov_row_kernels<R>([](auto k) { ELBA_HIP(hipFuncSetAttribute(reinterpret_cast<const void *>(k), hipFuncAttributeMaxDynamicSharedMemorySize, (int)OV_LDS_MAX)); }), ...);
}

static OvSpecParams ov_spec_params(const OvParams &p)
{
    OvSpecParams q{};
    q.a_rowptr = p.a_rowptr; q.a_csr = p.a_csr; q.a_ell = p.a_ell; q.tick_rows = p.tick_rows;
    q.s_stride = p.s_stride; q.lpc_log2 = p.lpc_log2; q.max_col = p.max_col; q.fbits = p.fbits; q.M = p.M; q.Mcols = p.Mcols; q.use_feedback = p.use_feedback;
    for (int t = 0; t < NUM_LDS_TIERS; ++t) q.tier_limit[t] = p.tier_limit[t];
    q.fb_enough = p.fb_enough; q.tmp_cap = p.tmp_cap;
    q.row_cnt = p.row_cnt; q.low_cnt = p.low_cnt; q.row_off = p.row_off; q.lists = p.lists; q.sample_list = p.sample_list; q.ctr = p.ctr;
    q.rec = p.rec; q.tick = p.tick; q.slab = p.slab; q.slab_pos = p.slab_pos;
    return q;
}

template <int R> static void ov_launch_row(const OvLaunch &l, const OvPlan &plan, const OvParams &p, hipStream_t s, uint32_t sample)
{
    constexpr OvTierRow r = OV_ROWS[R];
    const dim3 grid((unsigned)l.grid), block((unsigned)r.block);
    const uint32_t tb = (uint32_t)r.tbits;
    if constexpr (ov_row_has_spec<R>()) {
        if (plan.spec) { hipLaunchKernelGGL((ov_row_kernel<R, 0, true>()), grid, block, l.lds, s, ov_spec_params(p), r.tier, tb, sample); return; }
    }
    if (r.dense || plan.dk == 0) hipLaunchKernelGGL((ov_row_kernel<R, 0, false>()), grid, block, l.lds, s, p, r.tier, tb, sample);
    else if (plan.dk == 1) hipLaunchKernelGGL((ov_row_kernel<R, 1, false>()), grid, block, l.lds, s, p, r.tier, tb, sample);
    else if (plan.dk == 4) hipLaunchKernelGGL((ov_row_kernel<R, 4, false>()), grid, block, l.lds, s, p, r.tier, tb, sample);
    else hipLaunchKernelGGL((ov_row_kernel<R, 2, false>()), grid, block, l.lds, s, p, r.tier, tb, sample);
}
template <int... R> static void ov_launch(std::integer_sequence<int, R...>, const OvLaunch &l, const OvPlan &plan, const OvParams &p, hipStream_t s, uint32_t sample)
{
    ((l.row == R ? ov_launch_row<R>(l, plan, p, s, sample) : (void)0), ...);
}
using OvRowSeq = std::make_integer_sequence<int, OV_NROWS>;

struct OvRun {
    Ctx &c;
    OvInput in; OvPlan plan;
    OvParams p{};
    OvCounters *hc = nullptr;
    int passes = 0;
    bool timed = false, was_timed = true;
    float ms_sym = 0, ms_num = 0, ms_fin = 0, ms_tot = 0;
};

static void ov_bind(OvRun &r)
{
    Ctx &c = r.c;
    const OvPlan &pl = r.plan;
    const int64_t M = c.M;
    ++r.passes;
    const int stride = c.cfg.timing_stride > 1 ? c.cfg.timing_stride : 1;
    r.timed = r.passes > 1 || (c.ov_calls++ % (uint64_t)stride) == 0;
    c.ov_tmp_cap = pl.tmp_cap;
    c.ov_tmp.reserve((size_t)pl.tmp_cap * sizeof(StageRec));
    c.ov_rec16 = pl.mir16;
    c.b_cap_entries = pl.b_cap;
    c.b_col.reserve((size_t)(pl.b_cap + 1) * 4);
    c.b_val.reserve((size_t)(pl.b_cap + 1) * sizeof(elba_seed_t));
    if (pl.half) c.ov_mir.reserve((size_t)(pl.b_cap + 1) * (pl.mir16 ? 16 : sizeof(StageRec)));
    c.ov_slab_on = pl.slab_on;
    if (pl.slab_on) { c.ov_slab_cap = pl.slab_cap; c.ov_slab.reserve((size_t)pl.slab_cap * 16); c.ov_slabpos.reserve((size_t)(M + 4) * 8); c.ov_slabn.reserve((size_t)(M + 8) * 4); }
    c.ov_sample.reserve(OV_SAMPLE_ROWS * 4);

    OvParams &p = r.p;
    p = OvParams{};
    const RowWindow w = c.window();
    p.a_rowptr = c.a_rowptr.as<uint32_t>(); p.a_csr = c.a_csr.as<uint64_t>();
    p.a_ell = c.use_ell ? c.a_ell.as<uint64_t>() : nullptr; p.a_ellj = c.csr_suffix ? c.a_ellj.as<uint32_t>() : nullptr; p.j_shift = c.j_shift; p.dense_up = (uint32_t)c.opt.dense_up; p.a_colptr = c.a_colptr.as<uint32_t>(); p.a_csc = c.a_csc.as<uint64_t>();
    p.s_stride = c.s_stride; p.lpc_log2 = c.lpc_log2; p.max_col = pl.max_col;
    p.M = (uint32_t)M; p.Mcols = (uint32_t)M; p.row_lo = (uint32_t)w.lo; p.row_hi = (uint32_t)w.hi; p.fbits = c.fbits;
    p.half = pl.half; p.pos_mask = pl.pos_mask; p.hint_mask = pl.hint_mask; p.suffix = pl.suffix; p.inl = pl.inl;
    p.row_order = pl.row_order ? c.row_order.as<uint32_t>() : nullptr; p.row_label = pl.row_order ? c.row_label.as<uint32_t>() : nullptr;
    p.prior_q16 = pl.prior_q16; p.use_feedback = pl.use_feedback; p.fb_enough = pl.fb_enough;
    p.pay16 = pl.pay16 ? 1u : 0u; p.qblk_log2 = pl.qblk_log2; p.min_tier = pl.min_tier;
    for (int t = 0; t < NUM_LDS_TIERS; ++t) p.tier_limit[t] = pl.tier_limit[t];
    p.tick_rows = c.ov_tickrows.as<uint32_t>();
    p.row_cnt = c.ov_rowcnt.as<uint32_t>(); p.low_cnt = c.ov_totcnt.as<uint32_t>();
    p.row_off = c.ov_rowoff.as<unsigned long long>(); p.lists = c.ov_lists.as<uint32_t>();
    p.fin_lists = c.ov_lists.as<uint32_t>() + (size_t)NUM_TIERS * (size_t)(M + 1);
    p.ctr = c.ov_counters.as<OvCounters>();
    p.gtable = c.ov_gtable.as<uint32_t>(); p.gstride = pl.gstride;
    p.tmp = c.ov_tmp.as<StageRec>(); p.tmp_cap = (unsigned long long)pl.tmp_cap;
    p.rec16 = pl.mir16 ? 1u : 0u; p.rec = c.ov_tmp.as<uint4>(); p.tick = reinterpret_cast<uint32_t *>(c.ov_tmp.as<char>() + (size_t)pl.tmp_cap * 16);
    p.slab_prior_q16 = pl.slab_prior_q16; p.slab_pct = (uint32_t)c.opt.slab_pct;
    if (pl.slab_on) { p.slab = c.ov_slab.as<uint4>(); p.slab_cap = (unsigned long long)pl.slab_cap; p.slab_pos = c.ov_slabpos.as<unsigned long long>(); }
    p.nsample = pl.nsample; p.sstep = pl.sstep; p.sample_list = c.ov_sample.as<uint32_t>();
}

static OvRun ov_begin(Ctx &c, int phase)
{
    const int64_t M = c.M;
    accepted(c.v, phase == 0 ? EV_CREATE_SEED_MATRIX : phase == 1 ? EV_SEED_MATRIX_BEGIN : EV_SEED_MATRIX_SEND);
    c.ov_phase = 0;
    ELBA_REQUIRE(M < 0xFFFFFF00ll, ELBA_ERR_UNSUPPORTED, "read ids beyond 2^32 - 256 (the top of the id range marks empty slots and idle lanes)");
    if (c.cold_calls) { c.ov_prior_q16 = 0; c.ov_slab_q16 = 0; c.ov_tiers_known = false; c.ov_sort_used[0] = c.ov_sort_used[1] = true; }

    c.ov_rowcnt.reserve((size_t)(M + 2) * 4);
    c.ov_rowoff.reserve((size_t)(M + 1) * 8);
    c.ov_lists.reserve((size_t)(NUM_TIERS + 2) * (size_t)(M + 1) * 4);
    c.ov_counters.reserve(sizeof(OvCounters));
    c.b_rowptr.reserve((size_t)(M + 2) * 8);
    if (c.ov_totcnt.cap < (size_t)(M + 2) * 4) c.ov_low_clean = false;
    c.ov_totcnt.reserve((size_t)(M + 2) * 4);
    c.ov_tickrows.reserve((size_t)(M / 32 + 2) * 4);

    const OvSpill sp = ov_spill_tables(M, c.num_cus);
    c.ov_gtable.reserve((size_t)sp.blocks * 5 * sp.gstride * 4);
    OvRun r{c};
    r.in = ov_input(c, phase, 1);
    r.plan = plan_ov(r.in);
    ELBA_REQUIRE(!c.csr_inline || (c.use_ell && (phase >= 1 || r.plan.whole)), ELBA_ERR_STATE,
                 "this windowed matrix carries inline partners (option panel_inline): multiply it through elba_seed_matrix_send / _begin, or rebuild it without the option");
    c.ov_hints_used = r.plan.hints_used;
    static DeviceOnce attr_once;
    attr_once.run(c.device, [] { ov_set_attributes(OvRowSeq{}); });
    c.ov_host.reserve(sizeof(OvCounters));
    r.hc = static_cast<OvCounters *>(c.ov_host.p);
    *r.hc = OvCounters{};
    c.ov_passes = 0; c.ov_forwarded = 0; c.ov_spec = 0;
    ov_bind(r);
    return r;
}

static void ov_zero_counters(OvRun &r)
{
    Ctx &c = r.c;
    const int64_t M = c.M;
    if (r.timed) c.ov_marks.mark(0, c.stream);
    ZeroList z{};
    auto add = [&](void *ptr, size_t bytes) { z.p[z.n] = static_cast<uint32_t *>(ptr); z.words[z.n] = (bytes + 3) / 4; ++z.n; };
    if (!c.ov_low_clean) add(c.ov_totcnt.p, (size_t)(M + 2) * 4);
    add(c.ov_counters.p, sizeof(OvCounters));
    add(c.ov_rowcnt.p, (size_t)(M + 2) * 4);
    add(c.ov_tickrows.p, (size_t)(M / 32 + 2) * 4);
    if (r.plan.slab_on) add(c.ov_slabn.p, (size_t)(M + 8) * 4);
    size_t most = 0;
    for (int q = 0; q < z.n; ++q) most = std::max(most, z.words[q]);
    hipLaunchKernelGGL(k_zero_regions, dim3((unsigned)std::min<size_t>((most + 255) / 256, (size_t)r.plan.zero_blocks_max)), dim3(256), 0, c.stream, z);
    c.ov_low_clean = false;
}

static void ov_sample(OvRun &r)
{
    Ctx &c = r.c;
    const bool sampling = r.plan.sample.row >= 0;
    if (sampling) hipLaunchKernelGGL(k_classify_direct, dim3(1), dim3(256), 0, c.stream, r.p, 1);
    if (r.timed) c.ov_marks.mark(1, c.stream);
    if (!sampling) return;
    ov_launch(OvRowSeq{}, r.plan.sample, r.plan, r.p, c.stream, 1u);
    r.p.use_feedback = 0;
}

static void ov_classify(OvRun &r)
{
    if (r.plan.classify_blocks > 0) hipLaunchKernelGGL(k_classify_direct, dim3((unsigned)r.plan.classify_blocks), dim3(256), 0, r.c.stream, r.p, 0);
}

static void ov_numeric(OvRun &r)
{
    Ctx &c = r.c;
    c.ov_spec = r.plan.nrows > 0 && r.plan.spec ? 1 : 0;
    for (int t = 0; t < NUM_LDS_TIERS; ++t) c.ov_tier_limit[t] = (int64_t)r.plan.tier_limit[t];
    c.ov_family = (int64_t)r.plan.family; c.ov_pay16 = r.plan.pay16 ? 1 : 0; c.ov_rec16_used = r.plan.mir16 ? 1 : 0;
    for (int t = 0; t < NUM_TIERS; ++t)
        if ((r.plan.launched >> t) & 1u) ov_launch(OvRowSeq{}, r.plan.tier[t], r.plan, r.p, c.stream, 0u);
    if (r.plan.nrows > 0) ELBA_HIP(hipGetLastError());
    if (r.timed) c.ov_marks.mark(2, c.stream);
}

static void ov_finalize(Ctx &c, const OvFinPlan &fp, uint32_t half, const StageRec *remote, int64_t nremote, int64_t slot = 0)
{
    hipStream_t s = c.stream;
    const int64_t M = c.M;
    const RowWindow w = c.window();
    const int cus = c.num_cus;
    const bool mir16 = ov_mir16(c);
    c.ov_sortkeys.reserve((size_t)fp.huge_blocks * fp.sort_stride * 8);
    if (fp.scan_rowptr) c.ov_sum_tmp.reserve((size_t)(M + 2) * 4);
    FinParams f{};
    f.row_cnt = c.ov_rowcnt.as<uint32_t>(); f.low_cnt = c.ov_totcnt.as<uint32_t>(); f.tmp = c.ov_tmp.as<StageRec>(); f.mir = half ? c.ov_mir.as<StageRec>() : nullptr; f.half = half; f.row_off = c.ov_rowoff.as<unsigned long long>(); f.b_rowptr = c.b_rowptr.as<int64_t>();
    f.b_col = c.b_col.as<uint32_t>(); f.b_val = c.b_val.as<elba_seed_t>();
    f.M = (uint32_t)M; f.row_lo = (uint32_t)w.lo; f.row_hi = (uint32_t)w.hi; f.fin_lists = c.ov_lists.as<uint32_t>() + (size_t)NUM_TIERS * (size_t)(M + 1); f.ctr = c.ov_counters.as<OvCounters>();
    f.b_cap = c.b_cap_entries;
    f.mir16 = mir16 ? 1u : 0u;
    f.tick_rows = c.ov_tickrows.as<uint32_t>();
    f.rec16 = c.ov_rec16 ? 1u : 0u; f.rec = c.ov_tmp.as<uint4>(); f.tick = reinterpret_cast<const uint32_t *>(c.ov_tmp.as<char>() + (size_t)c.ov_tmp_cap * 16);
    f.a_rowptr = c.a_rowptr.as<uint32_t>(); f.slab = fp.slabs ? c.ov_slab.as<uint4>() : nullptr;
    f.slab_pos = f.slab ? c.ov_slabpos.as<unsigned long long>() : nullptr; f.slab_n = f.slab ? c.ov_slabn.as<uint32_t>() : nullptr;
    f.sortkeys = c.ov_sortkeys.as<uint64_t>(); f.sort_stride = fp.sort_stride;
    if (fp.slab_fold_blocks > 0) hipLaunchKernelGGL(k_slab_fold, dim3((unsigned)fp.slab_fold_blocks), dim3(256), 0, s, f);
    if (!fp.scan_rowptr) hipLaunchKernelGGL(k_row_pointers, dim3((unsigned)fp.rowptr_blocks), dim3(256), 0, s, f);
    else {
        f.sum_tmp = c.ov_sum_tmp.as<uint32_t>();
        hipLaunchKernelGGL(k_sum_counts, dim3((unsigned)fp.rowptr_blocks), dim3(256), 0, s, f);
        exclusive_scan_u32_to_i64(s, f.sum_tmp, c.b_rowptr.as<int64_t>(), M + 1, c.ws_scan);
    }
    if (fp.nrows <= 0) return;
    const dim3 rows((unsigned)fp.row_blocks);
    hipLaunchKernelGGL(k_mirror, rows, dim3(256), 0, s, f);
    if (nremote > 0 && slot == 0) hipLaunchKernelGGL(k_place_remote, dim3((unsigned)std::min<int64_t>((nremote + 255) / 256, (int64_t)cus * 32)), dim3(256), 0, s, f, remote, (unsigned long long)nremote, 0ull);
    if (nremote > 0 && slot != 0) hipLaunchKernelGGL(k_place_remote, dim3((unsigned)std::min<int64_t>((slot + 255) / 256, (int64_t)cus * 4), (unsigned)(nremote / slot)), dim3(256), 0, s, f, remote, (unsigned long long)nremote, (unsigned long long)slot);
    hipLaunchKernelGGL(k_finalize_wave, rows, dim3(256), 0, s, f);
    if (f.rec16 && f.mir16) hipLaunchKernelGGL(k_finalize_mid16, rows, dim3(256), 0, s, f);
    else hipLaunchKernelGGL(k_finalize_mid, rows, dim3(256), 0, s, f);
    if (fp.sorts & 1u) hipLaunchKernelGGL(k_finalize_bucket, dim3((unsigned)fp.bucket_blocks), dim3(256), 0, s, f);
    if (fp.sorts & 2u) hipLaunchKernelGGL(k_finalize_huge, dim3((unsigned)fp.huge_blocks), dim3(256), 0, s, f);
}

static void ov_read_back(OvRun &r)
{
    Ctx &c = r.c;
    if (r.timed) c.ov_marks.mark(3, c.stream);
    ELBA_HIP(hipMemcpyAsync(r.hc, c.ov_counters.p, sizeof(OvCounters), hipMemcpyDeviceToHost, c.stream));
    ELBA_HIP(hipStreamSynchronize(c.stream));
    if (r.timed) { r.ms_sym += c.ov_marks.ms(0, 1); r.ms_num += c.ov_marks.ms(1, 2); r.ms_fin = c.ov_marks.ms(2, 3); r.ms_tot += c.ov_marks.ms(0, 3); }
    r.was_timed = r.timed;
    c.ov_passes = r.passes; c.ov_forwarded += r.hc->nforward;
}

static bool ov_settle(OvRun &r)
{
    Ctx &c = r.c;
    const OvCounters &hc = *r.hc;
    const uint32_t sorts = r.in.phase == 0 ? r.plan.fin.sorts : 3u;
    bool missed = false;
    for (int t = 0; t < NUM_TIERS; ++t) missed |= !((r.plan.launched >> t) & 1u) && hc.tier_count[t] > 0;
    missed |= (!(sorts & 1u) && hc.fin_count[0] > 0) || (!(sorts & 2u) && hc.fin_count[1] > 0);
    if (!hc.overflow && !missed) { c.ov_low_clean = r.in.phase == 0; return true; }
    if (c.opt.trace) fprintf(stderr, "[elba] overlap call repeated: overflow=%u missed=%d cursor=%llu tmp_cap=%lld\n", hc.overflow, (int)missed, hc.cursor, (long long)c.ov_tmp_cap);
    ELBA_REQUIRE(r.passes < 4, ELBA_ERR_INTERNAL, "overlap output did not settle");
    c.ov_tiers_known = false;
    r.in = ov_next_pass(r.in, r.plan, hc.overflow != 0, hc.cursor);
    r.plan = plan_ov(r.in);
    ov_bind(r);
    return false;
}

static void ov_finish(Ctx &c, OvCounters &hc, int passes, bool was_timed, float ms_tot, float ms_sym, float ms_num, float ms_fin, int64_t extra_nnz, int64_t extra_upper)
{
    const int64_t M = c.M, N = c.N, Z = c.Z;
    const RowWindow w = c.window();
    elba_overlap_stats st{};
    st.nrows = w.rows();
#ifdef ELBA_PHASE_CLOCK
    fprintf(stderr, "[elba phase] wave-0 cycles summed over %llu workgroups: header=%llu init=%llu accumulate=%llu handoff=%llu sweep=%llu reserve=%llu store=%llu | rows %u,%u,%u,%u,%u,%u\n",
            hc.phase[10], hc.phase[0], hc.phase[1], hc.phase[2], hc.phase[3], hc.phase[4], hc.phase[5], hc.phase[6],
            hc.tier_count[0], hc.tier_count[1], hc.tier_count[2], hc.tier_count[3], hc.tier_count[4], hc.tier_count[5]);
#endif
    OvMeasured m;
    for (int sh = 0; sh < NUM_SHARDS; ++sh) {
        const OvShard &x = hc.shard[sh];
        hc.yraw += x.yraw; hc.nnz += x.nnz; hc.ndiag += x.ndiag; hc.nupper += x.nupper; hc.products += x.products;
        if (x.maxshared > hc.maxshared) hc.maxshared = x.maxshared;
        for (int t = 0; t < NUM_TIERS; ++t) hc.tier_done[t] += x.tier_done[t];
        m.fb_claims += x.fb_claims; m.fb_ub += x.fb_ub;
    }
    const int64_t Y = (int64_t)hc.nnz + extra_nnz;
    m.Z = Z; m.nnz = (int64_t)hc.nnz; m.ndiag = (int64_t)hc.ndiag; m.extra_nnz = extra_nnz; m.whole = w.lo == 0 && w.hi == M;
    for (int t = 0; t < NUM_TIERS; ++t) m.tier_count[t] = hc.tier_count[t];
    m.fin_count[0] = hc.fin_count[0]; m.fin_count[1] = hc.fin_count[1];
    OvHints old;
    old.prior_q16 = c.ov_prior_q16; old.slab_q16 = c.ov_slab_q16;
    const OvHints h = ov_next_hints(old, m);
    for (int t = 0; t < NUM_TIERS; ++t) c.ov_tier_used[t] = h.tier_used[t];
    c.ov_tiers_known = h.tiers_known;
    c.ov_sort_used[0] = h.sort_used[0]; c.ov_sort_used[1] = h.sort_used[1];
    c.ov_slab_q16 = h.slab_q16; c.ov_prior_q16 = h.prior_q16;
    c.ov_mir_placed = (int64_t)hc.mir_placed;
    for (int t = 0; t < NUM_TIERS; ++t) { c.ov_tier_queued[t] = (int64_t)hc.tier_count[t]; c.ov_tier_done[t] = (int64_t)hc.tier_done[t]; }
    c.ov_sort_rows[0] = (int64_t)hc.fin_count[0]; c.ov_sort_rows[1] = (int64_t)hc.fin_count[1];
    c.ov_slab_q16_used = hc.slab_q16;
    st.products = c.ov_hints_used ? c.A_products : (int64_t)hc.products;
    st.nnz_before_prune = (int64_t)hc.yraw;
    st.nnz = Y;
    st.nnz_diag = (int64_t)hc.ndiag;
    st.nnz_upper = (int64_t)hc.nupper + extra_upper;
    st.max_numshared = (int64_t)hc.maxshared;
    st.rows_lds = 0;
    for (int t = 0; t < NUM_LDS_TIERS; ++t) st.rows_lds += hc.tier_done[t];
    st.rows_global = (int64_t)hc.tier_done[NUM_LDS_TIERS];
    int64_t queued = 0;
    for (int t = 0; t < NUM_TIERS; ++t) queued += hc.tier_count[t];
// ... 275 lines not shown
```

elba_amd/csrc/spgemm_direct.hpp:

```cpp

enum : uint32_t { D_NEXT = 20, D_FB0 = 16, W_ACC_P = 54 , W_END2 = 56 };
constexpr uint32_t RING = 128;
constexpr uint32_t NOROW = 0xFFFFFFFFu, UNRESOLVED = 0xFFFFFFFEu;

__device__ __forceinline__ uint32_t wave_max_scan(uint32_t v)
{
    int x = (int)v, t;
    t = __builtin_amdgcn_update_dpp(0, x, 0x111 , 0xf, 0xf, false); x = t > x ? t : x;
    t = __builtin_amdgcn_update_dpp(0, x, 0x112 , 0xf, 0xf, false); x = t > x ? t : x;
    t = __builtin_amdgcn_update_dpp(0, x, 0x114 , 0xf, 0xf, false); x = t > x ? t : x;
    t = __builtin_amdgcn_update_dpp(0, x, 0x118 , 0xf, 0xf, false); x = t > x ? t : x;
    t = __builtin_amdgcn_update_dpp(0, x, 0x142 , 0xa, 0xf, false); x = t > x ? t : x;
    t = __builtin_amdgcn_update_dpp(0, x, 0x143 , 0xc, 0xf, false); x = t > x ? t : x;
    return (uint32_t)x;
}

__device__ __forceinline__ uint32_t wave_sum_dpp(uint32_t v)
{
    int x = (int)v;
    x += __builtin_amdgcn_update_dpp(0, x, 0x111 , 0xf, 0xf, false);
    x += __builtin_amdgcn_update_dpp(0, x, 0x112 , 0xf, 0xf, false);
    x += __builtin_amdgcn_update_dpp(0, x, 0x114 , 0xf, 0xf, false);
    x += __builtin_amdgcn_update_dpp(0, x, 0x118 , 0xf, 0xf, false);
    x += __builtin_amdgcn_update_dpp(0, x, 0x142 , 0xa, 0xf, false);
    x += __builtin_amdgcn_update_dpp(0, x, 0x143 , 0xc, 0xf, false);
    return (uint32_t)__builtin_amdgcn_readlane(x, 63);
}

__device__ __forceinline__ uint32_t wave_add_scan(uint32_t v)
{
    int x = (int)v;
    x += __builtin_amdgcn_update_dpp(0, x, 0x111 , 0xf, 0xf, false);
    x += __builtin_amdgcn_update_dpp(0, x, 0x112 , 0xf, 0xf, false);
    x += __builtin_amdgcn_update_dpp(0, x, 0x114 , 0xf, 0xf, false);
    x += __builtin_amdgcn_update_dpp(0, x, 0x118 , 0xf, 0xf, false);
    x += __builtin_amdgcn_update_dpp(0, x, 0x142 , 0xa, 0xf, false);
    x += __builtin_amdgcn_update_dpp(0, x, 0x143 , 0xc, 0xf, false);
    return (uint32_t)x;
}

__device__ __forceinline__ bool owns_pair(uint32_t i, uint32_t j, uint32_t row_lo, uint32_t row_hi, bool upper = false)
{
    return j < row_lo || j >= row_hi || (upper ? j > i : ((((i ^ j) & 1u) != 0u) ? j < i : j > i));
}

template <int BLOCK, bool GLOBAL, bool PAY, int DK = 2, bool SUFFIX = false, int TB = 0, bool SPEC = false>
__global__ __launch_bounds__(BLOCK, SUFFIX ? 8 : (DK == 4 ? 1 : 4)) void k_spgemm_direct(std::conditional_t<SPEC, OvSpecParams, OvParams> p, int tier, uint32_t lds_tbits, uint32_t sample)
{
    static_assert(!PAY || !GLOBAL, "payload accumulators: LDS tiers only");
    static_assert(!SPEC || (!GLOBAL && !PAY && !SUFFIX), "the reads path: LDS tiers, 32-bit accumulators carrying posT");
    extern __shared__ __attribute__((aligned(16))) uint32_t smem[];
    uint32_t *misc = GLOBAL ? smem : smem + (size_t)(PAY ? 6 : 4) * (1u << lds_tbits) + ((size_t)1 << lds_tbits) / 2;
    const uint32_t tid = threadIdx.x, lane = tid & 63;
    const uint64_t lt = (1ull << lane) - 1;
    const uint32_t nrows = sample ? p.ctr->sample_count : p.ctr->tier_count[tier];
    if (nrows == 0) return;
    const uint32_t lb = p.lpc_log2, sub = tid & ((1u << lb) - 1u), grp = tid >> lb, EPT = (uint32_t)BLOCK >> lb;
    const uint32_t fbits = p.fbits, fmask = (1u << fbits) - 1u, stride = p.s_stride;
    const bool ell = SPEC || p.a_ell != nullptr;
    const uint32_t hmask = p.hint_mask, pmask = p.pos_mask;
    const uint2 *csr2 = reinterpret_cast<const uint2 *>(p.a_csr);
    const uint32_t slab_q = (p.slab != nullptr && !sample) ? sfirst(p.ctr->slab_q16) : 0u;
    unsigned long long chunk_off = 0;
    uint32_t chunk_left = 0;
    auto w64 = [&](uint32_t k) { return reinterpret_cast<unsigned long long *>(&misc[k]); };
    if (tid >= 32 && tid < W_END2) misc[tid] = 0;
    if (tid >= D_FB0 && tid < D_FB0 + 4u) misc[tid] = 0;
    const uint32_t *queue = sample ? p.sample_list : p.lists + (size_t)tier * p.M;
    uint32_t qshard = blockIdx.x & 7u, qtried = 0;
    const uint32_t qb = p.qblk_log2;
    auto qplace = [&](uint32_t k) -> unsigned long long { return ((((unsigned long long)(k >> qb) * 8u + qshard) << qb) | (k & ((1u << qb) - 1u))); };
    auto draw = [&]() -> uint32_t { return atomicAdd(sample ? &p.ctr->sample_next[qshard][0] : &p.ctr->tier_next[tier][qshard][0], 1u); };
    auto resolve = [&](uint32_t k) -> uint32_t {
        for (;;) {
            const unsigned long long idx = qplace(k);
            if (idx < nrows) return queue[idx];
            if (++qtried >= 8u) return NOROW;
            qshard = (qshard + 1u) & 7u;
            k = draw();
        }
    };
    if (tid == 0) { const uint32_t r0 = resolve(draw()); misc[D_NEXT] = r0; if (r0 != NOROW) { misc[D_NEXT + 1] = p.a_rowptr[r0]; misc[D_NEXT + 2] = p.a_rowptr[r0 + 1]; } }
    auto init_table = [&]() {
        if (GLOBAL) return;
        const uint32_t T0 = 1u << lds_tbits;
        for (uint32_t s2 = tid; s2 < T0; s2 += BLOCK) {
            smem[s2] = EMPTY; smem[T0 + s2] = 0;
            if (PAY) { reinterpret_cast<unsigned long long *>(smem + 2 * T0)[s2] = ~0ull; reinterpret_cast<unsigned long long *>(smem + 2 * T0)[T0 + s2] = 0ull; }
            else { smem[2 * T0 + s2] = 0xFFFFFFFFu; smem[3 * T0 + s2] = 0; }
        }
        if (tid < 16) misc[tid] = 0;
    };
    init_table();
    uint32_t dpar = 0;
    __syncthreads();
    uint32_t fb_seen = 0;
    bool fb_settled = false;
#ifdef ELBA_PHASE_CLOCK
    unsigned long long ph[8] = {0, 0, 0, 0, 0, 0, 0, 0};
    unsigned long long tprev = __builtin_amdgcn_s_memtime();
#define ELBA_DSTAMP(k) do { const unsigned long long tn = __builtin_amdgcn_s_memtime(); ph[k] += tn - tprev; tprev = tn; } while (0)
#else
#define ELBA_DSTAMP(k) do { } while (0)
#endif

    uint32_t npar = 0;
    for (;;) {
        const uint32_t NB = D_NEXT + 4u * npar;
        npar ^= 1u;
        const uint32_t NBN = D_NEXT + 4u * npar;
        const uint32_t i = sfirst(misc[NB]);
        if (i == NOROW) break;
        uint32_t nidx = 0, nrow = UNRESOLVED, nrs = 0, nre = 0;
        if (tid == 0 && qtried < 8u) nidx = draw();
        const uint32_t rs = sfirst(misc[NB + 1]), nnz = sfirst(misc[NB + 2]) - rs;
        const unsigned long long prod_ub = (unsigned long long)nnz * p.max_col;
        const uint32_t ub_i = prod_ub < (unsigned long long)p.Mcols ? (uint32_t)prod_ub : p.Mcols;
        auto resolve_early = [&]() {
            if (tid == 0 && qtried < 8u) { const unsigned long long idx = qplace(nidx); if (idx < nrows) nrow = queue[idx]; }
        };
        auto bounds_early = [&]() { if (tid == 0 && nrow != UNRESOLVED && nrow != NOROW) { nrs = p.a_rowptr[nrow]; nre = p.a_rowptr[nrow + 1]; } };
        auto publish_next = [&]() {
            if (tid == 0) {
                const bool early = nrow != UNRESOLVED;
                if (!early) nrow = qtried < 8u ? resolve(nidx) : NOROW;
                if (nrow != NOROW && (!early || nre == 0)) { nrs = p.a_rowptr[nrow]; nre = p.a_rowptr[nrow + 1]; }
                misc[NBN] = nrow; misc[NBN + 1] = nrs; misc[NBN + 2] = nre;
                if (!GLOBAL) misc[3] = 0;
            }
        };

        if (!GLOBAL && p.use_feedback) {
            if (!fb_settled && (fb_seen < 4u || (fb_seen & 15u) == 0)) {
                if (tid == 0) {
                    const unsigned long long u = __hip_atomic_load(&p.ctr->fb_ub, __ATOMIC_RELAXED, __HIP_MEMORY_SCOPE_AGENT);
                    const unsigned long long c = __hip_atomic_load(&p.ctr->fb_claims, __ATOMIC_RELAXED, __HIP_MEMORY_SCOPE_AGENT);
                    misc[D_FB0] = (uint32_t)u; misc[D_FB0 + 1] = (uint32_t)(u >> 32); misc[D_FB0 + 2] = (uint32_t)c; misc[D_FB0 + 3] = (uint32_t)(c >> 32);
                }
                __syncthreads();
            }
            ++fb_seen;
            const unsigned long long gu = ((unsigned long long)misc[D_FB0 + 1] << 32) | misc[D_FB0], gc = ((unsigned long long)misc[D_FB0 + 3] << 32) | misc[D_FB0 + 2];
            fb_settled = gu >= p.fb_enough;
            if (gu >= (1ull << 18)) {
                const double pred = 1.25 * (double)nnz * (double)gc / (double)gu;
                const uint32_t gbits = guaranteed_tbits(ub_i, p.Mcols);
                if (pred > 1.2 * (double)p.tier_limit[tier] && gbits > lds_tbits) {
                    int t2 = tier + 1;
                    while (t2 < NUM_LDS_TIERS && pred > (double)p.tier_limit[t2]) ++t2;
                    if (t2 > (int)gbits - LDS_TBITS0) t2 = (int)gbits - LDS_TBITS0;
                    if (tid == 0) {
                        atomicAdd(&p.ctr->nforward, 1u);
                        const uint32_t at = atomicAdd(&p.ctr->tier_count[t2], 1u);
                        p.lists[(size_t)t2 * p.M + at] = i;
                    }
                    __syncthreads();
                    publish_next();
                    __syncthreads();
                    continue;
                }
            }
        }

        Table<GLOBAL> tab;
        tab.misc = misc;
        uint32_t *list = nullptr;
        uint16_t *list16 = nullptr;
        if (GLOBAL) {
            tab.tbits = guaranteed_tbits(ub_i, p.Mcols);
            tab.limit = 0xFFFFFFFFu;
            uint32_t *base = p.gtable + (size_t)blockIdx.x * 5 * p.gstride;
            tab.keys = base; tab.cnt = base + p.gstride; tab.smin = base + 2 * p.gstride; tab.smax = base + 3 * p.gstride;
            list = base + 4 * p.gstride;
        } else {
            tab.tbits = lds_tbits;
            const uint32_t T = 1u << lds_tbits;
            tab.limit = p.tier_limit[tier];
            tab.keys = smem; tab.cnt = smem + T; tab.smin = smem + 2 * T; tab.smax = smem + 3 * T;
            tab.vmin = reinterpret_cast<unsigned long long *>(smem + 2 * T); tab.vmax = tab.vmin + T;
            list16 = reinterpret_cast<uint16_t *>(smem + (PAY ? 6 : 4) * T);
        }
        const uint32_t T = tab.size();
        ELBA_DSTAMP(0);
        if (GLOBAL) {
            for (uint32_t s = tid; s < T; s += BLOCK) { tab.keys[s] = EMPTY; tab.cnt[s] = 0; tab.smin[s] = 0xFFFFFFFFu; tab.smax[s] = 0; }
            if (tid < 16) misc[tid] = 0;
            __syncthreads();
        }
        auto reset_slot = [&](uint32_t s2) {
            tab.keys[s2] = EMPTY; tab.cnt[s2] = 0;
            if (PAY) { tab.vmin[s2] = ~0ull; tab.vmax[s2] = 0ull; } else { tab.smin[s2] = 0xFFFFFFFFu; tab.smax[s2] = 0; }
        };
        const uint32_t DG = GLOBAL ? 0u : dpar;

        bool full = false;
        uint32_t dg = 0, pr = 0;
        uint32_t head = 0, tail = 0;
        const bool pay16 = !PAY && !SUFFIX && !GLOBAL && p.pay16 != 0u;
        uint32_t *qj = misc + 64 + (tid >> 6) * (SUFFIX ? 592u : (PAY ? 768u : (pay16 ? 512u : 640u)));
        uint32_t *qs = qj + RING;
        unsigned long long *qv = reinterpret_cast<unsigned long long *>(qj + RING);
        auto drain = [&](uint32_t n) {
            const uint32_t at = (head + lane) & (RING - 1u);
            const uint32_t j = qj[at];
            if (PAY) { const unsigned long long v = qv[at]; tab.insert_lds64(j, v, v, 1u, lane < n, full); }
            else { const uint32_t sq = qs[at]; tab.insert_lds(j, sq, sq, 1u, lane < n, full); }
            head += n;
        };
        auto slot = [&](uint32_t j, uint32_t posT, uint32_t seq, uint32_t posQ) {
            const uint64_t mv = __ballot(j != EMPTY);
            if (mv == 0) return;
            const uint64_t md = __ballot(j == i);
            pr += (uint32_t)__popcll(mv); dg += (uint32_t)__popcll(md);
            uint64_t mi = mv & ~md;
            if (p.half) mi &= __ballot(owns_pair(i, j, p.half == 2u ? 0u : p.row_lo, p.half == 2u ? 0xFFFFFFFFu : p.row_hi, !PAY && p.suffix != 0u));
            if (mi == 0) return;
            const bool ins = (mi >> lane) & 1ull;
            if (GLOBAL) { if (ins) tab.insert(j, seq, full); return; }
            const uint32_t at = (tail + (uint32_t)__popcll(mi & lt)) & (RING - 1u);
            if (ins) {
                qj[at] = j;
                if (PAY) qv[at] = ((unsigned long long)seq << 32) | (posQ << 16) | posT; else qs[at] = pay16 ? (seq << 16) | posT : seq;
            }
            tail += (uint32_t)__popcll(mi);
            if (tail - head >= 64u) drain(64u);
        };
        if (SUFFIX) {
            static_assert(!SUFFIX || !PAY, "dense path: 32-bit accumulators, the seeds of the few survivors are looked up");
            constexpr uint32_t UN = 2;
            static_assert(UN % 2 == 0, "windows of two batches");
            const uint32_t jsh = p.j_shift, Sj = 1u << jsh;
            const uint32_t il = p.row_label ? p.row_label[i] : i;
            const uint4 *ellq = reinterpret_cast<const uint4 *>(p.a_ellj);
            uint32_t *skid = qj + 2u * RING, *smeta = skid + 64, *spre = skid + 128, *sown = skid + 200;
            auto retry = [&](bool pred, uint32_t j, uint32_t sq1) {
                const uint64_t mm = __ballot(pred);
                if (mm == 0) return;
                const uint32_t at = (tail + __builtin_amdgcn_mbcnt_hi((uint32_t)(mm >> 32), __builtin_amdgcn_mbcnt_lo((uint32_t)mm, 0u))) & (RING - 1u);
                if (pred) { qj[at] = j; qs[at] = sq1; }
                tail += (uint32_t)__popcll(mm);
                if (tail - head >= 64u) drain(64u);
            };
#pragma unroll 1
            for (uint32_t cit = 0;; ++cit) {
                uint32_t cdraw = 0;
                if (lane == 0) { const uint32_t a14 = (uint32_t)(uintptr_t)&misc[14], step = 64u; asm volatile("ds_add_rtn_u32 %0, %1, %2\n\ts_waitcnt lgkmcnt(0)" : "=v"(cdraw) : "v"(a14), "v"(step) : "memory"); }
                const uint32_t cbase = sfirst(cdraw);
                if (cbase >= nnz) break;
                const bool valid = cbase + lane < nnz;
                const uint2 en = valid ? csr2[rs + cbase + lane] : make_uint2(0u, 0u);
                const uint32_t L = (en.x >> 23) & 127u, idx = (en.x >> 16) & 127u;
                const uint32_t w = valid ? L - idx - 1u : 0u;
                const uint32_t fs = Sj - w, p0 = fs >> 2;
                const uint32_t np = w ? (Sj >> 2) - p0 : 0u;
                const uint32_t inc = wave_add_scan(np);
                const uint32_t T = (uint32_t)__builtin_amdgcn_readlane((int)inc, 63);
                dg += (uint32_t)__popcll(__ballot(valid));
                __builtin_amdgcn_wave_barrier();
                skid[lane] = en.y; smeta[lane] = p0 | fs << 8 | L << 16; spre[lane] = inc - np;
                if (lane == 63) spre[64] = T;
                __builtin_amdgcn_fence(__ATOMIC_RELEASE, "wavefront");
                __builtin_amdgcn_wave_barrier();
                if (cit == 0) { resolve_early(); } else if (cit == 1) bounds_early();
#pragma unroll 1
                for (uint32_t base = 0; base < T; base += 64u * UN) {
                    uint4 x[UN];
                    uint32_t sq[UN], vr[UN];
                    bool ok[UN];
#pragma unroll
                    for (int hw = 0; hw < (int)UN / 2; ++hw) {
                        const uint32_t B = base + (uint32_t)hw * 128u;
                        sown[lane] = 0; sown[lane + 64u] = 0;
                        __builtin_amdgcn_wave_barrier();
                        if (np != 0u) {
                            const uint32_t pre = inc - np;
                            if (pre >= B && pre - B < 128u) sown[pre - B] = lane + 1u;
                            else if (pre < B && inc > B) sown[0] = lane + 1u;
                        }
                        __builtin_amdgcn_fence(__ATOMIC_ACQ_REL, "wavefront");
                        __builtin_amdgcn_wave_barrier();
                        const uint32_t m0 = wave_max_scan(sown[lane]);
                        const uint32_t carry = (uint32_t)__builtin_amdgcn_readlane((int)m0, 63);
                        uint32_t m1 = wave_max_scan(sown[lane + 64u]);
                        m1 = m1 > carry ? m1 : carry;
#pragma unroll
                        for (int v2 = 0; v2 < 2; ++v2) {
                            const int u = 2 * hw + v2;
                            const uint32_t c = B + (uint32_t)v2 * 64u + lane;
                            ok[u] = c < T;
                            const uint32_t en1 = v2 ? m1 : m0, lo = ok[u] ? en1 - 1u : 0u;
                            const uint32_t kl = skid[lo];
                            const uint32_t mt = smeta[lo], pc = (mt & 63u) + (c - spre[lo]), s0 = pc << 2, f0 = (mt >> 8) & 127u;
                            vr[u] = !ok[u] ? 4u : (f0 > s0 ? f0 - s0 : 0u);
                            sq[u] = ((cbase + lo) << fbits) + (s0 + (mt >> 16) - Sj);
                            x[u] = ok[u] ? ellq[((unsigned long long)kl << (jsh - 2u)) + pc] : make_uint4(EMPTY, EMPTY, EMPTY, EMPTY);
                        }
// ... 77 lines not shown
                }
                ft += (uint32_t)__popcll(mn);
                ea = eb; ca = cb;
                if (XC > 0) {
                    eb = ex[0]; cb = cx[0];
#pragma unroll
                    for (int q = 0; q + 1 < XC; ++q) { ex[q] = ex[q + 1]; cx[q] = cx[q + 1]; }
                    load_chunk(ex[XC > 0 ? XC - 1 : 0], cx[XC > 0 ? XC - 1 : 0]);
                } else load_chunk(eb, cb);
            };
            auto issue = [&](uint4 *x, uint32_t *pq, uint32_t *rk) {
#pragma unroll
                for (int u = 0; u < TR; ++u) {
                    const uint32_t k = (uint32_t)u * EW + gw;
                    x[u] = ones; pq[u] = 0; rk[u] = 0;
                    if (k < ft - fh && 2u * sub < stride) {
                        const uint32_t at = ((fh + k) & (FQ - 1u)) * (pay16 ? 2u : 3u);
                        if (pay16) { const uint32_t w0 = fq[at]; pq[u] = w0 & 0xFFFFu; rk[u] = w0 >> 16; }
                        else { pq[u] = fq[at]; rk[u] = fq[at + 2u]; }
                        x[u] = *reinterpret_cast<const uint4 *>(p.a_ell + ((unsigned long long)fq[at + 1u] * stride + 2u * sub));
                    }
                }
                const uint32_t n = ft - fh;
                fh += n < (uint32_t)TR * EW ? n : (uint32_t)TR * EW;
            };
            load_chunk(ea, ca); load_chunk(eb, cb);
#pragma unroll
            for (int q = 0; q < XC; ++q) load_chunk(ex[q], cx[q]);
            if (ca != NONE) consume();
            if (ca != NONE && ft - fh <= 64u) consume();
            uint4 x_cur[TR];
            uint32_t pq_cur[TR], rk_cur[TR];
            issue(x_cur, pq_cur, rk_cur);
#pragma unroll 1
            for (uint32_t it = 0;; ++it) {
#pragma unroll
                for (int u = 0; u < TR; ++u) asm volatile("" : "+v"(x_cur[u].x), "+v"(x_cur[u].y), "+v"(x_cur[u].z), "+v"(x_cur[u].w) : : "memory");
                asm volatile("" : "+v"(ea.x), "+v"(ea.y) : : "memory");
                if (ca != NONE && ft - fh <= 64u) consume();
                if (ca != NONE && ft - fh <= 64u) consume();
                const bool last = ft == fh && ca == NONE;
                uint4 x_nxt[TR];
                uint32_t pq_nxt[TR], rk_nxt[TR];
                issue(x_nxt, pq_nxt, rk_nxt);
                if (it == 0) resolve_early(); else if (it == 1) bounds_early();
#pragma unroll
                for (int u = 0; u < TR; ++u) {
                    const uint32_t seq = (rk_cur[u] << fbits) | (2u * sub);
                    slot(x_cur[u].y, x_cur[u].x, seq, pq_cur[u]);
                    slot(x_cur[u].w, x_cur[u].z, seq + 1u, pq_cur[u]);
                }
                if (tab.abandoned()) {
                    if (tid == 0) { const uint32_t done = ca != NONE ? ca : nnz; misc[11] = done < nnz ? done : nnz; }
                    break;
                }
                if (last) break;
#pragma unroll
                for (int u = 0; u < TR; ++u) { x_cur[u] = x_nxt[u]; pq_cur[u] = pq_nxt[u]; rk_cur[u] = rk_nxt[u]; }
            }
        } else if (!SUFFIX) {
#pragma unroll 1
            for (uint32_t t0 = 0; t0 < nnz; t0 += EPT) {
                const uint32_t r = t0 + grp;
                uint2 c = make_uint2(0u, 0u);
                uint32_t c0 = 0, len = 0;
                if (r < nnz) { c = csr2[rs + r]; if (!(c.x & hmask)) { c0 = p.a_colptr[c.y]; len = p.a_colptr[c.y + 1] - c0; } }
                if (hmask) dg += (uint32_t)__popcll(__ballot(sub == 0 && (c.x & hmask) != 0u));
#pragma unroll 1
                for (uint32_t b = 2u * sub; __ballot(b < len) != 0; b += 2u << lb) {
                    uint2 e0 = make_uint2(0u, EMPTY), e1 = e0;
                    if (b < len) e0 = reinterpret_cast<const uint2 *>(p.a_csc)[c0 + b];
                    if (b + 1u < len) e1 = reinterpret_cast<const uint2 *>(p.a_csc)[c0 + b + 1u];
                    const uint32_t seq = (r << fbits) | b;
                    slot(e0.y, e0.x, seq, c.x & pmask);
                    slot(e1.y, e1.x, seq + 1u, c.x & pmask);
                }
                if (tab.abandoned()) {
                    if (tid == 0) { const uint32_t done = t0 + EPT; misc[11] = done < nnz ? done : nnz; }
                    break;
                }
            }
        }
        if (!GLOBAL && tail != head) drain(tail - head);
        if ((pr | dg) != 0 && lane == 0) { lds_add32(&misc[DG], dg); lds_add32(&misc[12], pr); }
        ELBA_DSTAMP(2);
        publish_next();
        if (GLOBAL) __syncthreads(); else lds_barrier();
        ELBA_DSTAMP(3);
        if (tab.abandoned()) {
            if (tid == 0) {
                const uint32_t at = atomicAdd(&p.ctr->tier_count[tier + 1], 1u);
                p.lists[(size_t)(tier + 1) * p.M + at] = i;
                const unsigned long long all = nnz ? nnz : 1u, done = misc[11] ? misc[11] : all;
                lds_add64(w64(W_FB_C), (unsigned long long)misc[9] * all / done); lds_add64(w64(W_FB_U), (unsigned long long)nnz); lds_add32(&misc[W_FB_N], 1u);
                asm volatile("s_waitcnt lgkmcnt(0)" ::: "memory");
                if (p.use_feedback && misc[W_FB_N] >= 2 && ((((unsigned long long)misc[D_FB0 + 1] << 32) | misc[D_FB0]) < p.fb_enough)) {
                    const unsigned long long fc = *w64(W_FB_C), fu = *w64(W_FB_U);
                    atomicAdd(&p.ctr->fb_claims, fc); atomicAdd(&p.ctr->fb_ub, fu);
                    *w64(W_TOT_C) += fc; *w64(W_TOT_U) += fu; *w64(W_FB_C) = 0; *w64(W_FB_U) = 0; misc[W_FB_N] = 0;
                }
            }
            if (!GLOBAL) { __syncthreads(); init_table(); if (tid < 2) misc[tid] = 0; }
            __syncthreads();
            continue;
        }

        uint32_t yraw = 0;
        const bool relabel = SUFFIX && p.row_label != nullptr, whole = p.row_lo == 0u && p.row_hi == p.M;
        if (!GLOBAL && T == 4u * (uint32_t)BLOCK) {
            uint32_t jj[4], cc[4], pre[4], tot = 0;
            uint64_t bal[4];
#pragma unroll
            for (int u = 0; u < 4; ++u) { jj[u] = tab.keys[(uint32_t)u * BLOCK + tid]; cc[u] = tab.cnt[(uint32_t)u * BLOCK + tid]; }
            if (SUFFIX && relabel && !whole) {
#pragma unroll
                for (int u = 0; u < 4; ++u) if (jj[u] != EMPTY) jj[u] = p.row_order[jj[u]];
            }
#pragma unroll
            for (int u = 0; u < 4; ++u) {
                const uint32_t j = jj[u];
                if (j != EMPTY) yraw += (p.half == 2u || (p.half && j >= p.row_lo && j < p.row_hi)) ? 2u : 1u;
                bal[u] = __ballot(j != EMPTY && cc[u] >= 2u);
                if (j != EMPTY && cc[u] < 2u) reset_slot((uint32_t)u * BLOCK + tid);
                pre[u] = tot; tot += (uint32_t)__popcll(bal[u]);
            }
            if (tot) {
                uint32_t at = 0;
                if (lane == 0) asm volatile("ds_add_rtn_u32 %0, %1, %2\n\ts_waitcnt lgkmcnt(0)" : "=v"(at) : "v"((uint32_t)(uintptr_t)&misc[3]), "v"(tot) : "memory");
                at = sfirst(at);
#pragma unroll
                for (int u = 0; u < 4; ++u)
                    if ((bal[u] >> lane) & 1ull) list16[at + pre[u] + (uint32_t)__popcll(bal[u] & lt)] = (uint16_t)((uint32_t)u * BLOCK + tid);
            }
        } else
        for (uint32_t b0 = 0; b0 < T; b0 += BLOCK) {
            const uint32_t s0 = b0 + tid;
            bool keep = false;
            if (s0 < T) {
                uint32_t j = tab.ld(tab.keys, s0);
                if (j != EMPTY) {
                    if (SUFFIX && relabel && !whole) j = p.row_order[j];
                    yraw += (p.half == 2u || (p.half && j >= p.row_lo && j < p.row_hi)) ? 2u : 1u; keep = tab.ld(tab.cnt, s0) >= 2;
                    if (!GLOBAL && !keep) reset_slot(s0);
                }
            }
            const uint64_t bal = __ballot(keep);
            if (bal == 0) continue;
            uint32_t at = 0;
            if (lane == 0) at = atomicAdd(&misc[3], (uint32_t)__popcll(bal));
            at = __shfl(at, 0, 64) + (uint32_t)__popcll(bal & lt);
            if (keep) { if (GLOBAL) list[at] = s0; else list16[at] = (uint16_t)s0; }
        }
        yraw = wave_sum_dpp(yraw);
        if (lane == 0 && yraw) lds_add32(&misc[5], yraw);
        if (GLOBAL) __syncthreads(); else lds_barrier();
        ELBA_DSTAMP(4);
        if (tid == 0) {
            const uint32_t dcount = misc[DG];
            const uint32_t ytot = misc[3] + (dcount >= 2 ? 1u : 0u);
            unsigned long long off;
            if (ytot <= chunk_left) { off = chunk_off; chunk_off += ytot; chunk_left -= ytot; }
            else if (ytot >= STAGE_CHUNK / 2) off = atomicAdd(&p.ctr->cursor, (unsigned long long)ytot);
            else { off = atomicAdd(&p.ctr->cursor, (unsigned long long)STAGE_CHUNK); chunk_off = off + ytot; chunk_left = STAGE_CHUNK - ytot; }
            const bool fits = off + ytot <= p.tmp_cap;
            if (!fits) atomicOr(&p.ctr->overflow, 1u);
            p.row_cnt[i] = fits ? ytot : 0u;
            p.row_off[i] = off;
            misc[6] = (uint32_t)off; misc[7] = (uint32_t)(off >> 32); misc[8] = fits ? 1u : 0u;
            lds_add64(w64(W_ACC_YRAW), (unsigned long long)(misc[5] + (dcount >= 1 ? 1u : 0u)));
            lds_add64(w64(W_ACC_P), (unsigned long long)misc[12]);
            lds_add32(&misc[W_ACC_DONE], 1u);
            lds_add32(&misc[W_ACC_NDIAG], dcount >= 2 ? 1u : 0u);
            lds_add64(w64(W_ACC_Y), (unsigned long long)ytot);
            if (!GLOBAL) { lds_add64(w64(W_FB_C), (unsigned long long)misc[9]); lds_add64(w64(W_FB_U), (unsigned long long)nnz); lds_add32(&misc[W_FB_N], 1u); }
            if (p.use_feedback && misc[W_FB_N] >= 8 && ((((unsigned long long)misc[D_FB0 + 1] << 32) | misc[D_FB0]) < p.fb_enough)) {
                const unsigned long long fc = *w64(W_FB_C), fu = *w64(W_FB_U);
                atomicAdd(&p.ctr->fb_claims, fc); atomicAdd(&p.ctr->fb_ub, fu);
                *w64(W_TOT_C) += fc; *w64(W_TOT_U) += fu; *w64(W_FB_C) = 0; *w64(W_FB_U) = 0; misc[W_FB_N] = 0;
            }
        }
        lds_barrier();
        ELBA_DSTAMP(5);
        const uint32_t fits_row = misc[8], ysurv_row = misc[3], dcount_row = misc[DG];
        if (!GLOBAL && tid < 16 && tid != 3u && (tid < 6u ? tid == (DG ^ 1u) || tid == 5u : tid > 8u)) misc[tid] = 0;
        if (fits_row) {
            const unsigned long long off = ((unsigned long long)misc[7] << 32) | misc[6];
            const uint32_t ysurv = ysurv_row;
            const uint32_t hasd = dcount_row >= 2 ? 1u : 0u;
            uint32_t nup = 0, mx = 0, nmir = 0;
            bool drew = false;
            auto seed_at = [&](uint32_t a, uint32_t &q, uint32_t &t) {
                const uint2 ce = csr2[rs + (a >> fbits)];
                if (p.inl != 0u && (ce.y >> 31) != 0u) { q = ce.x & 0xFFFFu; t = ce.x >> 16; return; }
                q = ce.x & pmask;
                t = ell ? (uint32_t)p.a_ell[(unsigned long long)ce.y * stride + (a & fmask)] : (uint32_t)p.a_csc[p.a_colptr[ce.y] + (a & fmask)];
            };
            for (uint32_t t = tid; t < ysurv + hasd; t += BLOCK) {
                elba_seed_t v;
                uint32_t j = i;
                if (t < ysurv) {
                    const uint32_t s0 = GLOBAL ? __hip_atomic_load(&list[t], __ATOMIC_RELAXED, __HIP_MEMORY_SCOPE_AGENT) : (uint32_t)list16[t];
                    j = tab.ld(tab.keys, s0); v.numshared = (int32_t)tab.ld(tab.cnt, s0);
                    if (SUFFIX && relabel) j = p.row_order[j];
                    if (PAY) {
                        const uint32_t va = (uint32_t)tab.vmin[s0], vb = (uint32_t)tab.vmax[s0];
                        v.q0 = va >> 16; v.t0 = va & 0xFFFFu; v.q1 = vb >> 16; v.t1 = vb & 0xFFFFu;
                    } else if (pay16) {
                        const uint32_t va = tab.ld(tab.smin, s0), vb = tab.ld(tab.smax, s0);
                        const uint2 ca2 = csr2[rs + ((va >> 16) >> fbits)], cb2 = csr2[rs + ((vb >> 16) >> fbits)];
                        v.q0 = (p.inl != 0u && (ca2.y >> 31) != 0u) ? (ca2.x & 0xFFFFu) : (ca2.x & pmask); v.t0 = va & 0xFFFFu;
                        v.q1 = (p.inl != 0u && (cb2.y >> 31) != 0u) ? (cb2.x & 0xFFFFu) : (cb2.x & pmask); v.t1 = vb & 0xFFFFu;
                    } else {
                        seed_at(tab.ld(tab.smin, s0), v.q0, v.t0);
                        seed_at(tab.ld(tab.smax, s0), v.q1, v.t1);
                    }
                    if (!GLOBAL) reset_slot(s0);
                } else {
                    v.numshared = (int32_t)dcount_row;
                    const uint2 e0 = csr2[rs], e1 = csr2[rs + nnz - 1u];
                    v.q0 = v.t0 = (p.inl != 0u && (e0.y >> 31) != 0u) ? (e0.x & 0xFFFFu) : (e0.x & pmask);
                    v.q1 = v.t1 = (p.inl != 0u && (e1.y >> 31) != 0u) ? (e1.x & 0xFFFFu) : (e1.x & pmask);
                }
                uint32_t tick = 0xFFFFFFFFu;
                if (p.half && j != i && j >= p.row_lo && j < p.row_hi) {
                    ++nmir;
                    if (slab_q) {
                        const unsigned long long w = atomicAdd(&p.slab_pos[j], 1ull);
                        const uint32_t at = (uint32_t)w;
                        if (at < (uint32_t)(w >> 32)) p.slab[at] = make_uint4(i, v.t0 | v.q0 << 16, v.t1 | v.q1 << 16, (uint32_t)v.numshared);
                        else tick = atomicAdd(&p.low_cnt[j], 1u);
                    } else tick = atomicAdd(&p.low_cnt[j], 1u);
                }
                drew |= tick != 0xFFFFFFFFu;
                if (p.rec16) {
                    p.rec[off + t] = make_uint4(j, v.q0 | v.t0 << 16, v.q1 | v.t1 << 16, (uint32_t)v.numshared);
                    if (tick != 0xFFFFFFFFu) { const uint32_t at = atomicAdd(&p.ctr->ntick, 1u); p.tick[3ull * at] = i; p.tick[3ull * at + 1u] = t; p.tick[3ull * at + 2u] = tick; }
                }
                else {
                    p.tmp[off + t].a = make_uint4(j, tick, v.q0, v.t0);
                    p.tmp[off + t].b = make_uint4(v.q1, v.t1, (uint32_t)v.numshared, 0u);
                }
                if (j != i && ((p.half && j >= p.row_lo && j < p.row_hi) || j > i)) ++nup;
                mx = (uint32_t)v.numshared > mx ? (uint32_t)v.numshared : mx;
            }
            if (__ballot(drew) != 0 && lane == 0) atomicOr(&p.tick_rows[i >> 5], 1u << (i & 31u));
            if (nup) lds_add64(w64(W_NUP), (unsigned long long)nup);
            if (nmir) lds_add64(w64(W_MIR), (unsigned long long)nmir);
            if (mx) lds_max32(&misc[W_MX], mx);
        } else if (!GLOBAL) {
            for (uint32_t t = tid; t < ysurv_row; t += BLOCK) reset_slot((uint32_t)list16[t]);
        }
        dpar ^= 1u;
        if (GLOBAL) __syncthreads(); else lds_barrier();
// ... 111 lines not shown
```

elba_amd/csrc/spgemm_table.hpp:

```cpp
enum : uint32_t {
    W_ACC_YRAW = 32 , W_ACC_Y = 34 , W_ACC_DONE = 36, W_ACC_NDIAG = 37, W_FB_N = 38,
    W_FB_C = 40 , W_FB_U = 42 , W_TOT_C = 44 , W_TOT_U = 46 , W_NUP = 48 , W_MIR = 50 , W_MX = 52, W_END = 54
};
template <bool GLOBAL>
struct Table {
    uint32_t *keys, *cnt, *smin, *smax, *misc;
    unsigned long long *vmin, *vmax;
    uint32_t tbits, limit;
    __device__ __forceinline__ uint32_t size() const { return 1u << tbits; }
    __device__ __forceinline__ bool abandoned() const { return !GLOBAL && __hip_atomic_load(&misc[10], __ATOMIC_RELAXED, __HIP_MEMORY_SCOPE_WORKGROUP) != 0; }
    __device__ __forceinline__ void insert(uint32_t j, uint32_t s, bool &full) const
    {
        if (full) return;
        const uint32_t mask = size() - 1;
        uint32_t slot = (j * 0x9E3779B1u) >> (32 - tbits);
        for (;;) {
            const uint32_t k = atomicCAS(&keys[slot], EMPTY, j);
            if (k == j) break;
            if (k == EMPTY) {
                if (!GLOBAL) { if (atomicAdd(&misc[9], 1u) >= limit) { __hip_atomic_store(&misc[10], 1u, __ATOMIC_RELAXED, __HIP_MEMORY_SCOPE_WORKGROUP); full = true; } }
                break;
            }
            slot = (slot + 1) & mask;
        }
        atomicAdd(&cnt[slot], 1u);
        atomicMin(&smin[slot], s);
        atomicMax(&smax[slot], s);
    }
    __device__ __forceinline__ void insert_lds(uint32_t j, uint32_t s, uint32_t smx, uint32_t cnt, bool valid, bool &full) const
    {
        if (full) return;
        uint32_t slot = lds_slot(j);
        uint32_t claimed = 0, old, addr = 0;
        unsigned long long save, t;
        const uint32_t base = (uint32_t)(uintptr_t)keys;
        const uint32_t mask = size() - 1, empty = EMPTY;
        const uint32_t tb = size() * 4;
        if (valid) {
            asm volatile(
                "s_mov_b64 %[save], exec\n"
                ".Lprobe%=:\n\t"
                "v_lshl_add_u32 %[addr], %[slot], 2, %[base]\n\t"
                "ds_cmpst_rtn_b32 %[old], %[addr], %[empty], %[j]\n\t"
                "s_waitcnt lgkmcnt(0)\n\t"
                "v_cmp_eq_u32_e64 %[t], %[old], %[empty]\n\t"
                "v_cndmask_b32_e64 %[cl], %[cl], 1, %[t]\n\t"
                "v_cmp_eq_u32_e32 vcc, %[old], %[j]\n\t"
                "s_or_b64 vcc, vcc, %[t]\n\t"
                "s_andn2_b64 exec, exec, vcc\n\t"
                "s_cbranch_execz .Ldone%=\n\t"
                "v_add_u32_e32 %[slot], 1, %[slot]\n\t"
                "v_and_b32_e32 %[slot], %[mask], %[slot]\n\t"
                "s_branch .Lprobe%=\n"
                ".Ldone%=:\n\t"
                "s_mov_b64 exec, %[save]\n\t"
                "v_add_u32_e32 %[old], %[tb], %[addr]\n\t"
                "ds_add_u32 %[old], %[one]\n\t"
                "v_add_u32_e32 %[old], %[tb], %[old]\n\t"
                "ds_min_u32 %[old], %[s]\n\t"
                "v_add_u32_e32 %[old], %[tb], %[old]\n\t"
                "ds_max_u32 %[old], %[smx]\n"
                : [save] "=&s"(save), [addr] "+v"(addr), [old] "=&v"(old), [t] "=&s"(t), [cl] "+v"(claimed), [slot] "+v"(slot)
                : [base] "s"(base), [empty] "v"(empty), [j] "v"(j), [mask] "s"(mask), [tb] "s"(tb), [one] "v"(cnt), [s] "v"(s), [smx] "v"(smx)
                : "vcc", "memory");
        }
        if (__ballot(claimed != 0) != 0) {
            uint32_t prev = 0;
            if (claimed) {
                const uint32_t a9 = (uint32_t)(uintptr_t)&misc[9], one = 1u;
                asm volatile("ds_add_rtn_u32 %0, %1, %2\n\ts_waitcnt lgkmcnt(0)" : "=v"(prev) : "v"(a9), "v"(one) : "memory");
            }
            if (__ballot(claimed != 0 && prev >= limit) != 0) {
                misc[10] = 1u;
                full = true;
            }
        }
    }
    __device__ __forceinline__ void insert_lds64(uint32_t j, unsigned long long lo, unsigned long long hi, uint32_t cnt, bool valid, bool &full) const
    {
        if (full) return;
        uint32_t slot = lds_slot(j);
        uint32_t claimed = 0, old, addr = 0;
        unsigned long long save, t;
        const uint32_t base = (uint32_t)(uintptr_t)keys;
        const uint32_t base64 = (uint32_t)(uintptr_t)vmin;
        const uint32_t mask = size() - 1, empty = EMPTY;
        const uint32_t tb = size() * 4, tb8 = size() * 8;
        if (valid) {
            asm volatile(
                "s_mov_b64 %[save], exec\n"
                ".Lprobe%=:\n\t"
                "v_lshl_add_u32 %[addr], %[slot], 2, %[base]\n\t"
                "ds_cmpst_rtn_b32 %[old], %[addr], %[empty], %[j]\n\t"
                "s_waitcnt lgkmcnt(0)\n\t"
                "v_cmp_eq_u32_e64 %[t], %[old], %[empty]\n\t"
                "v_cndmask_b32_e64 %[cl], %[cl], 1, %[t]\n\t"
                "v_cmp_eq_u32_e32 vcc, %[old], %[j]\n\t"
                "s_or_b64 vcc, vcc, %[t]\n\t"
                "s_andn2_b64 exec, exec, vcc\n\t"
                "s_cbranch_execz .Ldone%=\n\t"
                "v_add_u32_e32 %[slot], 1, %[slot]\n\t"
                "v_and_b32_e32 %[slot], %[mask], %[slot]\n\t"
                "s_branch .Lprobe%=\n"
                ".Ldone%=:\n\t"
                "s_mov_b64 exec, %[save]\n\t"
                "v_add_u32_e32 %[old], %[tb], %[addr]\n\t"
                "ds_add_u32 %[old], %[one]\n\t"
                "v_lshl_add_u32 %[old], %[slot], 3, %[base64]\n\t"
                "ds_min_u64 %[old], %[lo]\n\t"
                "v_add_u32_e32 %[old], %[tb8], %[old]\n\t"
                "ds_max_u64 %[old], %[hi]\n"
                : [save] "=&s"(save), [addr] "+v"(addr), [old] "=&v"(old), [t] "=&s"(t), [cl] "+v"(claimed), [slot] "+v"(slot)
                : [base] "s"(base), [base64] "s"(base64), [empty] "v"(empty), [j] "v"(j), [mask] "s"(mask), [tb] "s"(tb), [tb8] "s"(tb8), [one] "v"(cnt), [lo] "v"(lo), [hi] "v"(hi)
                : "vcc", "memory");
        }
        if (__ballot(claimed != 0) != 0) {
            uint32_t prev = 0;
            if (claimed) {
                const uint32_t a9 = (uint32_t)(uintptr_t)&misc[9], one = 1u;
                asm volatile("ds_add_rtn_u32 %0, %1, %2\n\ts_waitcnt lgkmcnt(0)" : "=v"(prev) : "v"(a9), "v"(one) : "memory");
// ... 102 lines not shown
```

Measured before the change: 16.85 billion.

## Specialize overlap kernel on ELL geometry and fold row-count passes

Adds a GEOM-specialized variant of the spec overlap kernel. It is chosen when stride is 8, lpc is 4 and fbits is 3, and it turns table size, tier limit, stride and LDS offsets into compile-time constants for the hash insert asm. It also merges slab folding, count summation and wide-row queueing into one k_row_counts kernel (or the rowptr scan), which takes that work out of k_mirror. It drops the pair-count accumulation in the spec path. The cost is one more kernel instantiation, and the path only helps when the matrix geometry matches.

```diff
diff --git a/elba_amd/csrc/capi.hip b/elba_amd/csrc/capi.hip
--- a/elba_amd/csrc/capi.hip
+++ b/elba_amd/csrc/capi.hip
@@ -791,10 +791,11 @@
         ELBA_REQUIRE(name, ELBA_ERR_INVALID_ARG, "set_option: null name");
         struct { const char *n; bool *b; } flags[] = {
             {"overlap_cold_calls", &c.cold_calls}, {"no_symmetry", &c.opt.no_symmetry}, {"no_ell", &c.opt.no_ell}, {"no_pay", &c.opt.no_pay}, {"mir32", &c.opt.mir32},
-            {"no_hints", &c.opt.no_hints}, {"no_sample", &c.opt.no_sample}, {"no_slab", &c.opt.no_slab}, {"no_ell_compact", &c.opt.no_ell_compact}, {"msd_no_rank", &c.opt.msd_no_rank}, {"msd_rank", &c.opt.msd_rank}, {"csr_pairs_late", &c.opt.csr_pairs_late}, {"no_suffix", &c.opt.no_suffix}, {"ov_generic", &c.opt.ov_generic}, {"no_row_order", &c.opt.no_row_order}, {"no_inline", &c.opt.no_inline}, {"panel_inline", &c.opt.panel_inline}, {"kmer_pairs", &c.opt.kmer_pairs},
+            {"no_hints", &c.opt.no_hints}, {"no_sample", &c.opt.no_sample}, {"no_slab", &c.opt.no_slab}, {"no_ell_compact", &c.opt.no_ell_compact}, {"msd_no_rank", &c.opt.msd_no_rank}, {"msd_rank", &c.opt.msd_rank}, {"csr_pairs_late", &c.opt.csr_pairs_late}, {"no_suffix", &c.opt.no_suffix}, {"no_row_order", &c.opt.no_row_order}, {"no_inline", &c.opt.no_inline}, {"panel_inline", &c.opt.panel_inline}, {"kmer_pairs", &c.opt.kmer_pairs},
             {"kmer_unfused", &c.opt.kmer_unfused}, {"kmer_no_msd", &c.opt.kmer_no_msd}, {"kmer_msd", &c.opt.kmer_msd}, {"csr_pairs", &c.opt.csr_pairs}, {"emit_plain", &c.opt.emit_plain}, {"trace", &c.opt.trace}, {"measure_prep", &c.opt.measure_prep}};
         for (auto &f : flags) if (!strcmp(name, f.n)) { *f.b = value != 0; return; }
-        if (!strcmp(name, "kmer_drop")) { ELBA_REQUIRE(value >= 0 && value <= 3, ELBA_ERR_INVALID_ARG, "set_option: kmer_drop is 0..3"); c.opt.kmer_drop = (int)value; }
+        if (!strcmp(name, "ov_generic")) { ELBA_REQUIRE(value >= 0 && value <= 2, ELBA_ERR_INVALID_ARG, "set_option: ov_generic is 0, 1 or 2"); c.opt.ov_generic = value == 1; c.opt.ov_spec_rt_geom = value == 2; }
+        else if (!strcmp(name, "kmer_drop")) { ELBA_REQUIRE(value >= 0 && value <= 3, ELBA_ERR_INVALID_ARG, "set_option: kmer_drop is 0..3"); c.opt.kmer_drop = (int)value; }
         else if (!strcmp(name, "dense_up")) { ELBA_REQUIRE(value >= 0 && value <= 3, ELBA_ERR_INVALID_ARG, "set_option: dense_up is 0..3"); c.opt.dense_up = (int)value; }
         else if (!strcmp(name, "dense_wgs")) { ELBA_REQUIRE(value >= 1 && value <= 16, ELBA_ERR_INVALID_ARG, "set_option: dense_wgs is 1..16"); c.opt.dense_wgs = (int)value; }
         else if (!strncmp(name, "tune", 4) && name[4] >= '1' && name[4] <= '7' && name[4] != '6' && name[5] == 0) c.opt.tune[name[4] - '0'] = value;
@@ -857,6 +858,7 @@
         else if (!strcmp(name, "kmer_buckets")) *value = c.kmer_buckets;
         else if (!strcmp(name, "overlap_passes")) *value = c.ov_passes;
         else if (!strcmp(name, "overlap_spec")) *value = c.ov_spec;
+        else if (!strcmp(name, "overlap_spec_geom")) *value = c.ov_spec_geom;
         else if (!strcmp(name, "overlap_forwarded")) *value = c.ov_forwarded;
         else if (!strncmp(name, "overlap_tier_limit_", 19) && name[19] >= '0' && name[19] < '0' + NUM_LDS_TIERS && !name[20]) *value = c.ov_tier_limit[name[19] - '0'];
         else if (!strncmp(name, "overlap_tier_queued_", 20) && name[20] >= '0' && name[20] < '0' + NUM_TIERS && !name[21]) *value = c.ov_tier_queued[name[20] - '0'];
diff --git a/elba_amd/csrc/common.hpp b/elba_amd/csrc/common.hpp
--- a/elba_amd/csrc/common.hpp
+++ b/elba_amd/csrc/common.hpp
@@ -147,6 +147,7 @@
     bool no_inline = false;
     bool no_suffix = false;
     bool ov_generic = false;
+    bool ov_spec_rt_geom = false;
     bool no_row_order = false;
     bool kmer_pairs = false;
     bool kmer_unfused = false;
@@ -345,6 +346,7 @@
     bool ov_slab_on = false;
     uint32_t ov_slab_q16_used = 0;
     int64_t ov_mir_placed = 0;
+    int64_t ov_spec_geom = 0;
     int64_t ov_spec = 0;
     int64_t ov_tier_limit[5] = {0, 0, 0, 0, 0}, ov_tier_queued[6] = {0, 0, 0, 0, 0, 0}, ov_tier_done[6] = {0, 0, 0, 0, 0, 0}, ov_sort_rows[2] = {0, 0};
     int64_t ov_family = 0, ov_pay16 = 0, ov_rec16_used = 0;
diff --git a/elba_amd/csrc/ov_plan.hpp b/elba_amd/csrc/ov_plan.hpp
--- a/elba_amd/csrc/ov_plan.hpp
+++ b/elba_amd/csrc/ov_plan.hpp
@@ -20,6 +20,7 @@
 namespace ov_spec {
 constexpr uint32_t half = 1, inl = 1, pay16 = 1, rec16 = 1, suffix = 0, qblk_log2 = 0, j_shift = 0;
 constexpr uint32_t hint_mask = 1u << 31, pos_mask = 0x3FFFFFFFu;
+constexpr uint32_t geom_stride = 8, geom_lpc_log2 = 2, geom_fbits = 3;
 }
 
 enum OvFamily { OV_DENSE, OV_PAY, OV_S32, OV_SHARED };
@@ -45,6 +46,8 @@
 };
 constexpr int OV_NROWS = (int)(sizeof(OV_ROWS) / sizeof(OV_ROWS[0]));
 
+constexpr uint32_t ov_tier_limit(int tbits, int block) { return std::min(((1u << tbits) >> 2) * 3, (1u << tbits) - (uint32_t)block) - 1; }
+
 constexpr int64_t ov_stage_slack(int num_cus) { return (int64_t)num_cus * 32 * STAGE_CHUNK + 64; }
 
 constexpr size_t ov_row_lds(const OvTierRow &r, bool pay16)
@@ -65,13 +68,14 @@
 
 struct OvOptions {
     bool no_symmetry = false, no_pay = false, mir32 = false, no_slab = false, no_sample = false, ov_generic = false;
+    bool spec_rt_geom = false;
     int dk = -1, dense_up = 1, dense_wgs = 8, slab_q16 = 0, slab_pct = 175;
     int64_t tune3 = 0, tune4 = 0, tune5 = 0, tune7 = 0;
 };
 struct OvHints { uint32_t prior_q16 = 0, slab_q16 = 0; bool tiers_known = false, tier_used[NUM_TIERS] = {false, false, false, false, false, false}, sort_used[2] = {false, false}; };
 struct OvInput {
     int64_t M = 0, N = 0, Z = 0, row_lo = 0, row_hi = 0, max_row_nnz = 0, max_col_nnz = 0;
-    uint32_t fbits = 1;
+    uint32_t fbits = 1, s_stride = 0, lpc_log2 = 0;
     bool pos16 = false, use_ell = false, csr_hints = false, csr_inline = false, csr_suffix = false, have_row_order = false;
     int num_cus = 256;
     OvOptions opt;
@@ -90,13 +94,15 @@
 };
 struct OvPlan {
     int64_t nrows = 0;
+    bool geom_off = false;
     bool whole = false, ell = false, forced = false;
     uint32_t half = 0, pos_mask = 0, hint_mask = 0, suffix = 0, inl = 0;
     bool row_order = false, hints_used = false;
     bool pay = false, pay16 = false;
     OvFamily family = OV_S32;
     int dk = 1;
-    bool spec = false;
+    bool spec = false, spec_geom = false;
+    uint32_t s_stride = 0, lpc_log2 = 0, fbits = 0;
     uint32_t min_tier = 0, qblk_log2 = 0, prior_q16 = 16384, use_feedback = 1, max_col = 1;
     unsigned long long fb_enough = 0;
     uint32_t nsample = 0, sstep = 1;
@@ -117,6 +123,11 @@
     return !p.forced && p.dk == 0 && !p.pay && (p.pay16 ? 1u : 0u) == ov_spec::pay16 && p.ell && p.half == ov_spec::half && p.hint_mask == ov_spec::hint_mask &&
            p.pos_mask == ov_spec::pos_mask && p.inl == ov_spec::inl && (p.mir16 ? 1u : 0u) == ov_spec::rec16 && p.suffix == ov_spec::suffix && !p.row_order &&
            p.qblk_log2 == ov_spec::qblk_log2 && p.whole;
+}
+
+inline bool ov_spec_geom_ok(const OvPlan &p)
+{
+    return ov_spec_ok(p) && !p.geom_off && p.s_stride == ov_spec::geom_stride && p.lpc_log2 == ov_spec::geom_lpc_log2 && p.fbits == ov_spec::geom_fbits;
 }
 
 inline OvLaunch ov_launch_of(int row, bool pay16, int num_cus, int dense_wgs, int spill_blocks)
@@ -204,6 +215,7 @@
     if (o.tune7 >= 1 && o.tune7 <= NUM_TIERS) p.min_tier = (uint32_t)(o.tune7 - 1);
     p.dk = o.dk >= 0 ? o.dk : ((in.csr_inline && in.N > 0 && Z < 3 * in.N) ? 0 : 1);
     p.spec = ov_spec_ok(p);
+    p.spec_geom = ov_spec_geom_ok(p);
 }
 
 inline void ov_plan_sample_slabs(const OvInput &in, OvPlan &p)
@@ -226,10 +238,8 @@
     const OvOptions &o = in.opt;
     const int64_t M = in.M, nrows = p.nrows;
     for (int t = 0; t < NUM_TIERS; ++t) p.tier[t] = ov_launch_of(ov_row_of(p.family, t, (int)o.dense_up), p.pay16, in.num_cus, o.dense_wgs, p.spill_blocks);
-    for (int t = 0; t < NUM_LDS_TIERS; ++t) {
-        const uint32_t T = 1u << OV_ROWS[p.tier[t].row].tbits;
-        p.tier_limit[t] = std::min((T >> 2) * 3, T - (uint32_t)p.tier[t].block) - 1;
-    }
+    for (int t = 0; t < NUM_LDS_TIERS; ++t)
+        p.tier_limit[t] = ov_tier_limit(OV_ROWS[p.tier[t].row].tbits, p.tier[t].block);
     if (p.nsample) p.sample = p.tier[OV_SAMPLE_TIER];
     if (o.tune4 != 2 && in.pass == 1) {
         const uint64_t ubm = std::min<uint64_t>((uint64_t)std::max<int64_t>(in.max_row_nnz, 1) * (uint64_t)p.max_col, (uint64_t)(uint32_t)M);
@@ -251,6 +261,7 @@
     p.nrows = nrows;
     p.whole = in.row_lo == 0 && in.row_hi == in.M;
     p.ell = in.use_ell;
+    p.s_stride = in.s_stride; p.lpc_log2 = in.lpc_log2; p.fbits = in.fbits; p.geom_off = o.spec_rt_geom;
     p.forced = o.ov_generic || o.dk >= 0 || o.tune3 != 0 || o.tune4 != 0 || o.tune5 != 0 || o.tune7 != 0;
     ov_plan_capacities(in, p);
     ov_plan_switches(in, p);
diff --git a/elba_amd/csrc/spgemm.hip b/elba_amd/csrc/spgemm.hip
--- a/elba_amd/csrc/spgemm.hip
+++ b/elba_amd/csrc/spgemm.hip
@@ -145,6 +145,7 @@
     uint32_t *fin_lists; OvCounters *ctr;
     uint64_t *sortkeys; unsigned long long sort_stride;
     uint32_t *sum_tmp;
+    uint32_t queue_in_rowptr;
     long long b_cap;
     uint32_t mir16;
     const uint32_t *tick_rows;
@@ -164,18 +165,38 @@
     if (!s.q16) return make_uint2(0u, 0u);
     return make_uint2(slab_base(p.a_rowptr[i], s.rp0, i - p.row_lo, s.q16), p.slab_n[i]);
 }
-__global__ void k_slab_fold(FinParams p)
-{
-    const uint32_t i = p.row_lo + blockIdx.x * blockDim.x + threadIdx.x;
-    if (i >= p.row_hi) return;
-    const SlabCall s = slab_call(p);
-    uint32_t n = 0;
-    if (s.q16) {
-        const unsigned long long w = p.slab_pos[i];
-        const uint32_t base = slab_base(p.a_rowptr[i], s.rp0, i - p.row_lo, s.q16), cur = (uint32_t)w, lim = (uint32_t)(w >> 32);
-        n = (cur < lim ? cur : lim) - base;
-    }
-    p.slab_n[i] = n;
+__device__ __forceinline__ void fin_queue_wide(const FinParams &p, uint32_t i, uint32_t y)
+{
+    if (y <= FIN_WAVE2_MAX || i < p.row_lo || i >= p.row_hi) return;
+    const int which = y > FIN_LDS_MAX ? 1 : 0;
+    const uint32_t at = atomicAdd(&p.ctr->fin_count[which], 1u);
+    p.fin_lists[(size_t)which * p.M + at] = i;
+}
+
+__global__ __launch_bounds__(256) void k_row_counts(FinParams p)
+{
+    const uint32_t e = blockIdx.x * blockDim.x + threadIdx.x;
+    if (e > p.M) return;
+    uint32_t y = 0;
+    if (e < p.M) {
+        uint32_t n = 0;
+        if (p.slab_n) {
+            n = p.slab_n[e];
+            if (e >= p.row_lo && e < p.row_hi) {
+                const SlabCall s = slab_call(p);
+                n = 0;
+                if (s.q16) {
+                    const unsigned long long w = p.slab_pos[e];
+                    const uint32_t base = slab_base(p.a_rowptr[e], s.rp0, e - p.row_lo, s.q16), cur = (uint32_t)w, lim = (uint32_t)(w >> 32);
+                    n = (cur < lim ? cur : lim) - base;
+                }
+                p.slab_n[e] = n;
+            }
+        }
+        y = p.row_cnt[e] + p.low_cnt[e] + n;
+        fin_queue_wide(p, e, y);
+    }
+    if (p.sum_tmp) p.sum_tmp[e] = y;
 }
 
 __device__ __forceinline__ void fin_load(const FinParams &p, uint32_t low, unsigned long long off, int64_t dst, uint32_t t, uint4 &a, uint4 &b, uint2 sl = make_uint2(0u, 0u))
@@ -225,6 +246,7 @@
         const uint32_t e = t0 + tid * 4 + u;
         v[u] = e < p.M ? p.row_cnt[e] + p.low_cnt[e] + (p.slab_n ? p.slab_n[e] : 0u) : 0u;
         mine += v[u];
+        if (p.queue_in_rowptr && e < p.M) fin_queue_wide(p, e, v[u]);
     }
 #pragma unroll
     for (int d = 32; d >= 1; d >>= 1) pre += __shfl_xor(pre, d, 64);
@@ -246,28 +268,16 @@
     }
 }
 
-__global__ void k_sum_counts(FinParams p)
-{
-    const uint32_t e = blockIdx.x * blockDim.x + threadIdx.x;
-    if (e <= p.M) p.sum_tmp[e] = e < p.M ? p.row_cnt[e] + p.low_cnt[e] + (p.slab_n ? p.slab_n[e] : 0u) : 0u;
-}
-
 __global__ __launch_bounds__(256) void k_mirror(FinParams p)
 {
     const uint32_t lane = threadIdx.x & 63;
     const uint32_t wave = (blockIdx.x * blockDim.x + threadIdx.x) >> 6;
     const uint32_t nwaves = (gridDim.x * blockDim.x) >> 6;
     uint32_t placed = 0;
+    if (p.half && !p.rec16)
     for (uint32_t i = p.row_lo + wave; i < p.row_hi; i += nwaves) {
         const uint32_t own = p.row_cnt[i];
         const unsigned long long off = p.row_off[i];
-        const uint32_t y = own + p.low_cnt[i] + (p.slab_n ? p.slab_n[i] : 0u);
-        if (lane == 0 && y > FIN_WAVE2_MAX) {
-            const int which = y > FIN_LDS_MAX ? 1 : 0;
-            const uint32_t at = atomicAdd(&p.ctr->fin_count[which], 1u);
-            p.fin_lists[(size_t)which * p.M + at] = i;
-        }
-        if (!p.half || p.rec16) continue;
         if (p.tick_rows && !((p.tick_rows[i >> 5] >> (i & 31u)) & 1u)) continue;
         for (uint32_t t = lane; t < own; t += 64) {
             const uint4 a = p.tmp[off + t].a;
@@ -714,10 +724,10 @@
     OvInput in;
     const RowWindow w = c.window();
     in.M = c.M; in.N = c.N; in.Z = c.Z; in.row_lo = w.lo; in.row_hi = w.hi; in.max_row_nnz = c.max_row_nnz; in.max_col_nnz = c.max_col_nnz;
-    in.fbits = c.fbits; in.pos16 = c.pos16; in.use_ell = c.use_ell; in.csr_hints = c.csr_hints; in.csr_inline = c.csr_inline; in.csr_suffix = c.csr_suffix;
+    in.fbits = c.fbits; in.s_stride = c.use_ell ? c.s_stride : 0u; in.lpc_log2 = c.lpc_log2; in.pos16 = c.pos16; in.use_ell = c.use_ell; in.csr_hints = c.csr_hints; in.csr_inline = c.csr_inline; in.csr_suffix = c.csr_suffix;
     in.have_row_order = c.have_row_order; in.num_cus = c.num_cus;
     const Options &o = c.opt;
-    in.opt.no_symmetry = o.no_symmetry; in.opt.no_pay = o.no_pay; in.opt.mir32 = o.mir32; in.opt.no_slab = o.no_slab; in.opt.no_sample = o.no_sample; in.opt.ov_generic = o.ov_generic;
+    in.opt.no_symmetry = o.no_symmetry; in.opt.no_pay = o.no_pay; in.opt.mir32 = o.mir32; in.opt.no_slab = o.no_slab; in.opt.no_sample = o.no_sample; in.opt.ov_generic = o.ov_generic; in.opt.spec_rt_geom = o.ov_spec_rt_geom;
     in.opt.dk = o.dk; in.opt.dense_up = o.dense_up; in.opt.dense_wgs = o.dense_wgs; in.opt.slab_q16 = o.slab_q16; in.opt.slab_pct = o.slab_pct;
     in.opt.tune3 = o.tune[3]; in.opt.tune4 = o.tune[4]; in.opt.tune5 = o.tune[5]; in.opt.tune7 = o.tune[7];
     in.hints.prior_q16 = c.ov_prior_q16; in.hints.slab_q16 = c.ov_slab_q16; in.hints.tiers_known = c.ov_tiers_known;
@@ -733,10 +743,11 @@
     return in;
 }
 
-template <int R, int DK, bool SPEC> static constexpr auto ov_row_kernel()
+template <int R, int DK, bool SPEC, bool GEOM = false> static constexpr auto ov_row_kernel()
 {
     constexpr OvTierRow r = OV_ROWS[R];
     if constexpr (r.dense) return &k_spgemm_direct<r.block, false, false, 2, true, r.tbc>;
+    else if constexpr (SPEC && GEOM) return &k_spgemm_direct<r.block, false, false, 0, false, r.tbits, true, true>;
     else if constexpr (SPEC) return &k_spgemm_direct<r.block, false, false, 0, false, 0, true>;
     else return &k_spgemm_direct<r.block, r.global, r.payload, DK>;
 }
@@ -745,7 +756,7 @@
 {
     f(ov_row_kernel<R, 0, false>());
     if constexpr (!OV_ROWS[R].dense) { f(ov_row_kernel<R, 1, false>()); f(ov_row_kernel<R, 2, false>()); f(ov_row_kernel<R, 4, false>()); }
-    if constexpr (ov_row_has_spec<R>()) f(ov_row_kernel<R, 0, true>());
+    if constexpr (ov_row_has_spec<R>()) { f(ov_row_kernel<R, 0, true>()); f(ov_row_kernel<R, 0, true, true>()); }
 }
 template <int... R> static void ov_set_attributes(std::integer_sequence<int, R...>)
 {
@@ -770,6 +781,7 @@
     const dim3 grid((unsigned)l.grid), block((unsigned)r.block);
     const uint32_t tb = (uint32_t)r.tbits;
     if constexpr (ov_row_has_spec<R>()) {
+        if (plan.spec_geom) { hipLaunchKernelGGL((ov_row_kernel<R, 0, true, true>()), grid, block, l.lds, s, ov_spec_params(p), r.tier, tb, sample); return; }
         if (plan.spec) { hipLaunchKernelGGL((ov_row_kernel<R, 0, true>()), grid, block, l.lds, s, ov_spec_params(p), r.tier, tb, sample); return; }
     }
     if (r.dense || plan.dk == 0) hipLaunchKernelGGL((ov_row_kernel<R, 0, false>()), grid, block, l.lds, s, p, r.tier, tb, sample);
@@ -867,7 +879,7 @@
     c.ov_host.reserve(sizeof(OvCounters));
     r.hc = static_cast<OvCounters *>(c.ov_host.p);
     *r.hc = OvCounters{};
-    c.ov_passes = 0; c.ov_forwarded = 0; c.ov_spec = 0;
+    c.ov_passes = 0; c.ov_forwarded = 0; c.ov_spec = 0; c.ov_spec_geom = 0;
     ov_bind(r);
     return r;
 }
@@ -910,6 +922,7 @@
 {
     Ctx &c = r.c;
     c.ov_spec = r.plan.nrows > 0 && r.plan.spec ? 1 : 0;
+    c.ov_spec_geom = r.plan.nrows > 0 && r.plan.spec_geom ? 1 : 0;
     for (int t = 0; t < NUM_LDS_TIERS; ++t) c.ov_tier_limit[t] = (int64_t)r.plan.tier_limit[t];
     c.ov_family = (int64_t)r.plan.family; c.ov_pay16 = r.plan.pay16 ? 1 : 0; c.ov_rec16_used = r.plan.mir16 ? 1 : 0;
     for (int t = 0; t < NUM_TIERS; ++t)
@@ -938,16 +951,15 @@
     f.a_rowptr = c.a_rowptr.as<uint32_t>(); f.slab = fp.slabs ? c.ov_slab.as<uint4>() : nullptr;
     f.slab_pos = f.slab ? c.ov_slabpos.as<unsigned long long>() : nullptr; f.slab_n = f.slab ? c.ov_slabn.as<uint32_t>() : nullptr;
     f.sortkeys = c.ov_sortkeys.as<uint64_t>(); f.sort_stride = fp.sort_stride;
-    if (fp.slab_fold_blocks > 0) hipLaunchKernelGGL(k_slab_fold, dim3((unsigned)fp.slab_fold_blocks), dim3(256), 0, s, f);
+    f.sum_tmp = fp.scan_rowptr ? c.ov_sum_tmp.as<uint32_t>() : nullptr;
+    const bool counts = fp.scan_rowptr || fp.slab_fold_blocks > 0;
+    f.queue_in_rowptr = counts ? 0u : 1u;
+    if (counts) hipLaunchKernelGGL(k_row_counts, dim3((unsigned)((M + 1 + 255) / 256)), dim3(256), 0, s, f);
     if (!fp.scan_rowptr) hipLaunchKernelGGL(k_row_pointers, dim3((unsigned)fp.rowptr_blocks), dim3(256), 0, s, f);
-    else {
-        f.sum_tmp = c.ov_sum_tmp.as<uint32_t>();
-        hipLaunchKernelGGL(k_sum_counts, dim3((unsigned)fp.rowptr_blocks), dim3(256), 0, s, f);
-        exclusive_scan_u32_to_i64(s, f.sum_tmp, c.b_rowptr.as<int64_t>(), M + 1, c.ws_scan);
-    }
+    else exclusive_scan_u32_to_i64(s, f.sum_tmp, c.b_rowptr.as<int64_t>(), M + 1, c.ws_scan);
     if (fp.nrows <= 0) return;
     const dim3 rows((unsigned)fp.row_blocks);
-    hipLaunchKernelGGL(k_mirror, rows, dim3(256), 0, s, f);
+    if (half) hipLaunchKernelGGL(k_mirror, f.rec16 ? dim3((unsigned)std::min<int>(fp.row_blocks, cus)) : rows, dim3(256), 0, s, f);
     if (nremote > 0 && slot == 0) hipLaunchKernelGGL(k_place_remote, dim3((unsigned)std::min<int64_t>((nremote + 255) / 256, (int64_t)cus * 32)), dim3(256), 0, s, f, remote, (unsigned long long)nremote, 0ull);
     if (nremote > 0 && slot != 0) hipLaunchKernelGGL(k_place_remote, dim3((unsigned)std::min<int64_t>((slot + 255) / 256, (int64_t)cus * 4), (unsigned)(nremote / slot)), dim3(256), 0, s, f, remote, (unsigned long long)nremote, (unsigned long long)slot);
     hipLaunchKernelGGL(k_finalize_wave, rows, dim3(256), 0, s, f);
diff --git a/elba_amd/csrc/spgemm_direct.hpp b/elba_amd/csrc/spgemm_direct.hpp
--- a/elba_amd/csrc/spgemm_direct.hpp
+++ b/elba_amd/csrc/spgemm_direct.hpp
@@ -44,19 +44,22 @@
     return j < row_lo || j >= row_hi || (upper ? j > i : ((((i ^ j) & 1u) != 0u) ? j < i : j > i));
 }
 
-template <int BLOCK, bool GLOBAL, bool PAY, int DK = 2, bool SUFFIX = false, int TB = 0, bool SPEC = false>
-__global__ __launch_bounds__(BLOCK, SUFFIX ? 8 : (DK == 4 ? 1 : 4)) void k_spgemm_direct(std::conditional_t<SPEC, OvSpecParams, OvParams> p, int tier, uint32_t lds_tbits, uint32_t sample)
+template <int BLOCK, bool GLOBAL, bool PAY, int DK = 2, bool SUFFIX = false, int TB = 0, bool SPEC = false, bool GEOM = false>
+__global__ __launch_bounds__(BLOCK, SUFFIX ? 8 : (DK == 4 ? 1 : 4)) void k_spgemm_direct(std::conditional_t<SPEC, OvSpecParams, OvParams> p, int tier, uint32_t lds_tbits_arg, uint32_t sample)
 {
     static_assert(!PAY || !GLOBAL, "payload accumulators: LDS tiers only");
     static_assert(!SPEC || (!GLOBAL && !PAY && !SUFFIX), "the reads path: LDS tiers, 32-bit accumulators carrying posT");
+    static_assert(!GEOM || (SPEC && TB >= LDS_TBITS0 && TB < LDS_TBITS0 + NUM_LDS_TIERS && (1 << TB) >= 2 * BLOCK), "compiled geometry: the reads path on an LDS tier whose size is a template argument");
+    constexpr int CTB = GEOM ? TB : 0;
+    const uint32_t lds_tbits = GEOM ? (uint32_t)TB : lds_tbits_arg;
     extern __shared__ __attribute__((aligned(16))) uint32_t smem[];
     uint32_t *misc = GLOBAL ? smem : smem + (size_t)(PAY ? 6 : 4) * (1u << lds_tbits) + ((size_t)1 << lds_tbits) / 2;
     const uint32_t tid = threadIdx.x, lane = tid & 63;
     const uint64_t lt = (1ull << lane) - 1;
     const uint32_t nrows = sample ? p.ctr->sample_count : p.ctr->tier_count[tier];
     if (nrows == 0) return;
-    const uint32_t lb = p.lpc_log2, sub = tid & ((1u << lb) - 1u), grp = tid >> lb, EPT = (uint32_t)BLOCK >> lb;
-    const uint32_t fbits = p.fbits, fmask = (1u << fbits) - 1u, stride = p.s_stride;
+    const uint32_t lb = GEOM ? ov_spec::geom_lpc_log2 : p.lpc_log2, sub = tid & ((1u << lb) - 1u), grp = tid >> lb, EPT = (uint32_t)BLOCK >> lb;
+    const uint32_t fbits = GEOM ? ov_spec::geom_fbits : p.fbits, fmask = (1u << fbits) - 1u, stride = GEOM ? ov_spec::geom_stride : p.s_stride;
     const bool ell = SPEC || p.a_ell != nullptr;
     const uint32_t hmask = p.hint_mask, pmask = p.pos_mask;
     const uint2 *csr2 = reinterpret_cast<const uint2 *>(p.a_csr);
@@ -145,7 +148,7 @@
             if (gu >= (1ull << 18)) {
                 const double pred = 1.25 * (double)nnz * (double)gc / (double)gu;
                 const uint32_t gbits = guaranteed_tbits(ub_i, p.Mcols);
-                if (pred > 1.2 * (double)p.tier_limit[tier] && gbits > lds_tbits) {
+                if (pred > 1.2 * (double)(GEOM ? ov_tier_limit(GEOM ? TB : 1, BLOCK) : p.tier_limit[tier]) && gbits > lds_tbits) {
                     int t2 = tier + 1;
                     while (t2 < NUM_LDS_TIERS && pred > (double)p.tier_limit[t2]) ++t2;
                     if (t2 > (int)gbits - LDS_TBITS0) t2 = (int)gbits - LDS_TBITS0;
@@ -175,7 +178,7 @@
         } else {
             tab.tbits = lds_tbits;
             const uint32_t T = 1u << lds_tbits;
-            tab.limit = p.tier_limit[tier];
+            tab.limit = GEOM ? ov_tier_limit(GEOM ? TB : 1, BLOCK) : p.tier_limit[tier];
             tab.keys = smem; tab.cnt = smem + T; tab.smin = smem + 2 * T; tab.smax = smem + 3 * T;
             tab.vmin = reinterpret_cast<unsigned long long *>(smem + 2 * T); tab.vmax = tab.vmin + T;
             list16 = reinterpret_cast<uint16_t *>(smem + (PAY ? 6 : 4) * T);
@@ -204,14 +207,15 @@
             const uint32_t at = (head + lane) & (RING - 1u);
             const uint32_t j = qj[at];
             if (PAY) { const unsigned long long v = qv[at]; tab.insert_lds64(j, v, v, 1u, lane < n, full); }
-            else { const uint32_t sq = qs[at]; tab.insert_lds(j, sq, sq, 1u, lane < n, full); }
+            else { const uint32_t sq = qs[at]; tab.template insert_lds<CTB>(j, sq, sq, 1u, lane < n, full); }
             head += n;
         };
         auto slot = [&](uint32_t j, uint32_t posT, uint32_t seq, uint32_t posQ) {
             const uint64_t mv = __ballot(j != EMPTY);
             if (mv == 0) return;
             const uint64_t md = __ballot(j == i);
-            pr += (uint32_t)__popcll(mv); dg += (uint32_t)__popcll(md);
+            if (!SPEC) pr += (uint32_t)__popcll(mv);
+            dg += (uint32_t)__popcll(md);
             uint64_t mi = mv & ~md;
             if (p.half) mi &= __ballot(owns_pair(i, j, p.half == 2u ? 0u : p.row_lo, p.half == 2u ? 0xFFFFFFFFu : p.row_hi, !PAY && p.suffix != 0u));
             if (mi == 0) return;
@@ -455,7 +459,7 @@
             }
         }
         if (!GLOBAL && tail != head) drain(tail - head);
-        if ((pr | dg) != 0 && lane == 0) { lds_add32(&misc[DG], dg); lds_add32(&misc[12], pr); }
+        if ((pr | dg) != 0 && lane == 0) { lds_add32(&misc[DG], dg); if (!SPEC) lds_add32(&misc[12], pr); }
         ELBA_DSTAMP(2);
         publish_next();
         if (GLOBAL) __syncthreads(); else lds_barrier();
@@ -480,7 +484,7 @@
 
         uint32_t yraw = 0;
         const bool relabel = SUFFIX && p.row_label != nullptr, whole = p.row_lo == 0u && p.row_hi == p.M;
-        if (!GLOBAL && T == 4u * (uint32_t)BLOCK) {
+        if (CTB ? (1u << CTB) == 4u * (uint32_t)BLOCK : (!GLOBAL && T == 4u * (uint32_t)BLOCK)) {
             uint32_t jj[4], cc[4], pre[4], tot = 0;
             uint64_t bal[4];
 #pragma unroll
@@ -541,7 +545,7 @@
             p.row_off[i] = off;
             misc[6] = (uint32_t)off; misc[7] = (uint32_t)(off >> 32); misc[8] = fits ? 1u : 0u;
             lds_add64(w64(W_ACC_YRAW), (unsigned long long)(misc[5] + (dcount >= 1 ? 1u : 0u)));
-            lds_add64(w64(W_ACC_P), (unsigned long long)misc[12]);
+            if (!SPEC) lds_add64(w64(W_ACC_P), (unsigned long long)misc[12]);
             lds_add32(&misc[W_ACC_DONE], 1u);
             lds_add32(&misc[W_ACC_NDIAG], dcount >= 2 ? 1u : 0u);
             lds_add64(w64(W_ACC_Y), (unsigned long long)ytot);
diff --git a/elba_amd/csrc/spgemm_table.hpp b/elba_amd/csrc/spgemm_table.hpp
--- a/elba_amd/csrc/spgemm_table.hpp
+++ b/elba_amd/csrc/spgemm_table.hpp
@@ -27,15 +27,75 @@
         atomicMin(&smin[slot], s);
         atomicMax(&smax[slot], s);
     }
+    template <int CTB = 0>
     __device__ __forceinline__ void insert_lds(uint32_t j, uint32_t s, uint32_t smx, uint32_t cnt, bool valid, bool &full) const
     {
         if (full) return;
-        uint32_t slot = lds_slot(j);
+        uint32_t slot = CTB ? (j * 0x9E3779B1u) >> (32 - (CTB ? CTB : 1)) : lds_slot(j);
         uint32_t claimed = 0, old, addr = 0;
         unsigned long long save, t;
         const uint32_t base = (uint32_t)(uintptr_t)keys;
         const uint32_t mask = size() - 1, empty = EMPTY;
         const uint32_t tb = size() * 4;
+        if constexpr (CTB != 0) {
+            static_assert(CTB == 0 || (CTB >= 9 && CTB <= 13), "LDS tiers: 512 .. 8192 slots");
+            constexpr bool NEAR = (12u << CTB) <= 0xFFFFu;
+            static_assert((4u << CTB) <= 0xFFFFu, "the count array lies within the 16-bit offset field");
+            if (valid) {
+                if constexpr (NEAR) {
+                    asm volatile(
+                        "s_mov_b64 %[save], exec\n"
+                        ".Lprobe%=:\n\t"
+                        "v_lshl_add_u32 %[addr], %[slot], 2, %[base]\n\t"
+                        "ds_cmpst_rtn_b32 %[old], %[addr], %[empty], %[j]\n\t"
+                        "s_waitcnt lgkmcnt(0)\n\t"
+                        "v_cmp_eq_u32_e64 %[t], %[old], %[empty]\n\t"
+                        "v_cndmask_b32_e64 %[cl], %[cl], 1, %[t]\n\t"
+                        "v_cmp_eq_u32_e32 vcc, %[old], %[j]\n\t"
+                        "s_or_b64 vcc, vcc, %[t]\n\t"
+                        "s_andn2_b64 exec, exec, vcc\n\t"
+                        "s_cbranch_execz .Ldone%=\n\t"
+                        "v_add_u32_e32 %[slot], 1, %[slot]\n\t"
+                        "v_and_b32_e32 %[slot], %[mask], %[slot]\n\t"
+                        "s_branch .Lprobe%=\n"
+                        ".Ldone%=:\n\t"
+                        "s_mov_b64 exec, %[save]\n\t"
+                        "ds_add_u32 %[addr], %[one] offset:%[o1]\n\t"
+                        "ds_min_u32 %[addr], %[s] offset:%[o2]\n\t"
+                        "ds_max_u32 %[addr], %[smx] offset:%[o3]\n"
+                        : [save] "=&s"(save), [addr] "+v"(addr), [old] "=&v"(old), [t] "=&s"(t), [cl] "+v"(claimed), [slot] "+v"(slot)
+                        : [base] "s"(base), [empty] "v"(empty), [j] "v"(j), [mask] "n"((1u << CTB) - 1u), [one] "v"(cnt), [s] "v"(s), [smx] "v"(smx),
+                          [o1] "n"(NEAR ? (4u << CTB) : 0u), [o2] "n"(NEAR ? (8u << CTB) : 0u), [o3] "n"(NEAR ? (12u << CTB) : 0u)
+                        : "vcc", "memory");
+                } else {
+                    asm volatile(
+                        "s_mov_b64 %[save], exec\n"
+                        ".Lprobe%=:\n\t"
+                        "v_lshl_add_u32 %[addr], %[slot], 2, %[base]\n\t"
+                        "ds_cmpst_rtn_b32 %[old], %[addr], %[empty], %[j]\n\t"
+                        "s_waitcnt lgkmcnt(0)\n\t"
+                        "v_cmp_eq_u32_e64 %[t], %[old], %[empty]\n\t"
+                        "v_cndmask_b32_e64 %[cl], %[cl], 1, %[t]\n\t"
+                        "v_cmp_eq_u32_e32 vcc, %[old], %[j]\n\t"
+                        "s_or_b64 vcc, vcc, %[t]\n\t"
+                        "s_andn2_b64 exec, exec, vcc\n\t"
+                        "s_cbranch_execz .Ldone%=\n\t"
+                        "v_add_u32_e32 %[slot], 1, %[slot]\n\t"
+                        "v_and_b32_e32 %[slot], %[mask], %[slot]\n\t"
+                        "s_branch .Lprobe%=\n"
+                        ".Ldone%=:\n\t"
+                        "s_mov_b64 exec, %[save]\n\t"
+                        "ds_add_u32 %[addr], %[one] offset:%[o1]\n\t"
+                        "v_add_u32_e32 %[old], %[tb2], %[addr]\n\t"
+                        "ds_min_u32 %[old], %[s]\n\t"
+                        "ds_max_u32 %[old], %[smx] offset:%[o1]\n"
+                        : [save] "=&s"(save), [addr] "+v"(addr), [old] "=&v"(old), [t] "=&s"(t), [cl] "+v"(claimed), [slot] "+v"(slot)
+                        : [base] "s"(base), [empty] "v"(empty), [j] "v"(j), [mask] "n"((1u << CTB) - 1u), [tb2] "s"(8u << CTB), [one] "v"(cnt), [s] "v"(s), [smx] "v"(smx),
+                          [o1] "n"(4u << CTB)
+                        : "vcc", "memory");
+                }
+            }
+        } else
         if (valid) {
             asm volatile(
                 "s_mov_b64 %[save], exec\n"
```

Result: faster. 17.10 billion (median of 6 runs) (+1.5%).
